# PJLab-ADG/neuralsim

Hardware: NVIDIA H100
Metric: Mrays/sec fwd+bwd (higher is better)
Workload: dtype f16

## Files before the change

neuralsim_b200/csrc/color_tc.cu:

```cuda
#include "fused_tc_common.cuh"
#include "sh_device.cuh"

namespace nsb {

struct ColorNetDev {
    DecoderDevTC dec;
    const __half *R1, *rb1, *R2, *rb2, *R3, *rb3;
    int rw, rin, n_appear;
    float fac[3];
};

constexpr int XW = 64;
constexpr int kTileBytes = kTile * XW * 2;
constexpr int kChunk = kTile * 16;

__host__ __device__ inline int ref_col(int k, int n_appear) {
    if (k < 32) return 22 + k;
    if (k < 35) return k - 32;
    if (k < 51) return 3 + (k - 35);
    if (k < 54) return 19 + (k - 51);
    if (k < 54 + n_appear) return k;
    return -1;
}


__device__ __forceinline__ void level_jacobian(const PLMeta &m, uint32_t p, const float (&xs)[3], const __half *__restrict__ grid,
                                               float (&J0)[3], float (&J1)[3]) {
    uint32_t cell[8];
    float w[8], fr[3], scale[3];
    level_cells3(m, p, xs, cell, w, fr, scale);
    const uint32_t *lp = level_cells_ptr(m, p, grid);
    float2 v[8];
#pragma unroll
    for (int c = 0; c < 8; ++c) {
        const uint32_t raw = ld_nc_u32(lp + cell[c]);
        v[c] = __half22float2(*reinterpret_cast<const __half2 *>(&raw));
    }
#pragma unroll
    for (int gd = 0; gd < 3; ++gd) {
        float a0 = 0.f, a1 = 0.f;
#pragma unroll
        for (int c = 0; c < 4; ++c) {
            float ww = scale[gd];
            int left = 0;
#pragma unroll
            for (int k = 0; k < 2; ++k) {
                const int d = k >= gd ? k + 1 : k;
                if (c & (1 << k)) { ww = __fmul_rn(ww, fr[d]); left += 1 << d; }
                else ww = __fmul_rn(ww, __fsub_rn(1.f, fr[d]));
            }
            const int right = left + (1 << gd);
            a0 = __fmaf_rn(ww, __fsub_rn(v[right].x, v[left].x), a0);
            a1 = __fmaf_rn(ww, __fsub_rn(v[right].y, v[left].y), a1);
        }
        J0[gd] = a0;
        J1[gd] = a1;
    }
}

__device__ __forceinline__ void unpack8(const uint4 &q, float (&v)[8]) {
    const __half2 *h = reinterpret_cast<const __half2 *>(&q);
#pragma unroll
    for (int i = 0; i < 4; ++i) { const float2 f = __half22float2(h[i]); v[2 * i] = f.x; v[2 * i + 1] = f.y; }
}

constexpr int kColorGatherU = 4;

constexpr int kColorBwdCtasPerSM = 2;

__global__ void __launch_bounds__(kTile)
k_color_fwd(const PLMeta m, const __half *__restrict__ grid, const ColorNetDev net, const PointSrc ps, const float *__restrict__ view_dirs,
            const float *__restrict__ h_appear, int64_t n, int max_level, float *__restrict__ sdf_out, float *__restrict__ nab_out,
            float *__restrict__ rgb_out, float *__restrict__ x_out, uint8_t *__restrict__ Zt, uint8_t *__restrict__ Xt,
            uint8_t *__restrict__ Y1t, uint8_t *__restrict__ Y2t, const OccCollect oc, const int64_t *__restrict__ n_dev) {
    n = eff_n(n, n_dev);
    extern __shared__ uint8_t dyn_smem[];
    uint8_t *tiles = reinterpret_cast<uint8_t *>((reinterpret_cast<uintptr_t>(dyn_smem) + 1023) & ~uintptr_t(1023));
    uint8_t *sX = tiles;
    uint8_t *sU = sX + kTileBytes;
    uint8_t *sW1 = sU + kTileBytes;
    uint8_t *sW1T = sW1 + HW * NF * 2;
    uint8_t *sR1 = sW1T + HW * NF * 2;
    uint8_t *sR2 = sR1 + XW * XW * 2;
    constexpr int kS = tc::acc_stride(64);
    float *acc = reinterpret_cast<float *>(sR2 + XW * XW * 2);
    __shared__ float sb1[HW], sW2[HW], srb1[XW], srb2[XW], sR3[3][XW];
    __shared__ float sb2, srb3[3];

    const int tid = threadIdx.x;
    stage_W1(net.dec, sW1, tid);
    stage_W1T(net.dec, sW1T, tid);
    for (int e = tid; e < XW * XW; e += kTile) {
        const int j = e % XW, k = e / XW;
        const int rc = ref_col(k, net.n_appear);
        const __half v1 = (j < net.rw && rc >= 0) ? net.R1[j * net.rin + rc] : __float2half_rn(0.f);
        const __half v2 = (j < net.rw && k < net.rw) ? net.R2[j * net.rw + k] : __float2half_rn(0.f);
        *reinterpret_cast<__half *>(sR1 + (k / 8) * (XW * 16) + j * 16 + (k % 8) * 2) = v1;
        *reinterpret_cast<__half *>(sR2 + (k / 8) * (XW * 16) + j * 16 + (k % 8) * 2) = v2;
    }
    stage_decoder_vectors(net.dec, sb1, sW2, &sb2, tid);
    if (tid < XW) {
        srb1[tid] = tid < net.rw ? __half2float(net.rb1[tid]) : 0.f;
        srb2[tid] = tid < net.rw ? __half2float(net.rb2[tid]) : 0.f;
#pragma unroll
        for (int k = 0; k < 3; ++k) sR3[k][tid] = tid < net.rw ? __half2float(net.R3[k * net.rw + tid]) : 0.f;
    }
    if (tid == 0) {
        for (int k = 0; k < 3; ++k) srb3[k] = __half2float(net.rb3[k]);
    }
    tc::fence_async_smem();
    __syncthreads();
    const uint32_t x_addr = tc::smem_u32(sX), u_addr = tc::smem_u32(sU), w1_addr = tc::smem_u32(sW1), w1t_addr = tc::smem_u32(sW1T);
    const uint32_t r1_addr = tc::smem_u32(sR1), r2_addr = tc::smem_u32(sR2);
    const SoftplusK spk(net.dec.beta);

    const int64_t n_tiles = (n + kTile - 1) / kTile;
    for (int64_t tile = blockIdx.x; tile < n_tiles; tile += gridDim.x) {
        const int64_t i = tile * kTile + tid;
        const bool valid = i < n;
        float xn[3], xs[3];
        int64_t ray;
        load_point(ps, ps.x == nullptr, i, valid, xn, xs, ray);
        gather_row_to_tile<kTile, kColorGatherU>(m, grid, xs, max_level, sX, tid);
        tc::fence_async_smem();
        __syncthreads();
        tc::mma_to_rows<64, 0, 0, NF / 16>(acc, kS, 0, tc::kmajor(x_addr, kTile), tc::kmajor(w1_addr, HW), false);
        __syncthreads();
        float out = 0.f;
        uint8_t *zt = Zt ? Zt + tile * kTileBytes : nullptr;
#pragma unroll 1
        for (int c = 0; c < HW / 8; ++c) {
            float z[8], uu[8];
            tc::acc_ld8(acc, kS, tid, c * 8, z);
#pragma unroll
            for (int j = 0; j < 8; ++j) {
                z[j] = r16(z[j] + sb1[c * 8 + j]);
                float a, s;
                softplus_as(z[j], spk, a, s);
                out = fmaf(r16(a), sW2[c * 8 + j], out);
                uu[j] = sW2[c * 8 + j] * s;
            }
            *reinterpret_cast<uint4 *>(sU + c * kChunk + tid * 16) = tc::pack8_f16(uu);
            if (zt) *reinterpret_cast<uint4 *>(zt + c * kChunk + tid * 16) = tc::pack8_f16(z);
        }
        const float sdf = r16(out + sb2);
        tc::fence_async_smem();
        __syncthreads();
        tc::mma_to_rows<32, 0, 0, HW / 16>(acc, kS, 0, tc::kmajor(u_addr, kTile), tc::kmajor(w1t_addr, NF), false);
        __syncthreads();
        float nacc[3] = {0.f, 0.f, 0.f};
#pragma unroll 1
        for (uint32_t g4 = 0; g4 < 4; ++g4) {
            float gg[8];
            tc::acc_ld8(acc, kS, tid, g4 * 8, gg);
#pragma unroll
            for (uint32_t q = 0; q < 4; ++q) {
                const uint32_t p = g4 * 4 + q;
                if ((int)m.level[p] <= max_level) {
                    float J0[3], J1[3];
                    level_jacobian(m, p, xs, grid, J0, J1);
                    const float g0 = r16(gg[2 * q]), g1 = r16(gg[2 * q + 1]);
#pragma unroll
                    for (int d = 0; d < 3; ++d) nacc[d] = __fmaf_rn(g0, J0[d], nacc[d]);
#pragma unroll
                    for (int d = 0; d < 3; ++d) nacc[d] = __fmaf_rn(g1, J1[d], nacc[d]);
                }
            }
        }
        float nab[3];
#pragma unroll
        for (int d = 0; d < 3; ++d) nab[d] = __fmul_rn(__fmul_rn(nacc[d], 0.5f), net.fac[d]);
        {
            float xr[32];
#pragma unroll
            for (int k = 0; k < 32; ++k) xr[k] = 0.f;
            xr[0] = xn[0]; xr[1] = xn[1]; xr[2] = xn[2];
            if (valid) {
                sh_basis(view_dirs[ray * 3], view_dirs[ray * 3 + 1], view_dirs[ray * 3 + 2], 4, xr + 3);
                if (h_appear) {
#pragma unroll
                    for (int k = 0; k < 8; ++k)
                        if (k < net.n_appear) xr[22 + k] = h_appear[ray * net.n_appear + k];
                }
            }
#pragma unroll
            for (int d = 0; d < 3; ++d) xr[19 + d] = fminf(fmaxf(nab[d], -1.f), 1.f);
            uint8_t *xt = Xt ? Xt + tile * kTileBytes : nullptr;
#pragma unroll
            for (int c = 0; c < 4; ++c) {
                float v8[8];
#pragma unroll
                for (int k = 0; k < 8; ++k) v8[k] = xr[c * 8 + k];
                const uint4 q = tc::pack8_f16(v8);
                *reinterpret_cast<uint4 *>(sX + (4 + c) * kChunk + tid * 16) = q;
                if (xt) {
                    *reinterpret_cast<uint4 *>(xt + (4 + c) * kChunk + tid * 16) = q;
                    *reinterpret_cast<uint4 *>(xt + c * kChunk + tid * 16) = *reinterpret_cast<const uint4 *>(sX + c * kChunk + tid * 16);
                }
            }
        }
        tc::fence_async_smem();
        __syncthreads();
        tc::mma_to_rows<64, 0, 0, XW / 16>(acc, kS, 0, tc::kmajor(x_addr, kTile), tc::kmajor(r1_addr, XW), false);
        __syncthreads();
        uint8_t *y1t = Y1t ? Y1t + tile * kTileBytes : nullptr;
#pragma unroll 1
        for (int c = 0; c < XW / 8; ++c) {
            float y[8];
            tc::acc_ld8(acc, kS, tid, c * 8, y);
#pragma unroll
            for (int j = 0; j < 8; ++j) y[j] = fmaxf(r16(y[j] + srb1[c * 8 + j]), 0.f);
            const uint4 q = tc::pack8_f16(y);
            *reinterpret_cast<uint4 *>(sU + c * kChunk + tid * 16) = q;
            if (y1t) *reinterpret_cast<uint4 *>(y1t + c * kChunk + tid * 16) = q;
        }
        tc::fence_async_smem();
        __syncthreads();
        tc::mma_to_rows<64, 0, 0, XW / 16>(acc, kS, 0, tc::kmajor(u_addr, kTile), tc::kmajor(r2_addr, XW), false);
        __syncthreads();
        float o3[3] = {0.f, 0.f, 0.f};
        uint8_t *y2t = Y2t ? Y2t + tile * kTileBytes : nullptr;
#pragma unroll 1
        for (int c = 0; c < XW / 8; ++c) {
            float y[8];
            tc::acc_ld8(acc, kS, tid, c * 8, y);
#pragma unroll
            for (int j = 0; j < 8; ++j) {
                y[j] = fmaxf(r16(y[j] + srb2[c * 8 + j]), 0.f);
#pragma unroll
                for (int k = 0; k < 3; ++k) o3[k] = fmaf(y[j], sR3[k][c * 8 + j], o3[k]);
            }
            if (y2t) *reinterpret_cast<uint4 *>(y2t + c * kChunk + tid * 16) = tc::pack8_f16(y);
        }
        if (valid) {
            sdf_out[i] = sdf;
            if (oc.pcl) occ_collect_point(oc, xs, sdf);
#pragma unroll
            for (int d = 0; d < 3; ++d) {
                nab_out[i * 3 + d] = nab[d];
                const float y3 = r16(o3[d] + srb3[d]);
                rgb_out[i * 3 + d] = r16(1.f / (1.f + expf(-y3)));
                if (x_out) x_out[i * 3 + d] = xn[d];
            }
        }
        __syncthreads();
    }
}

__global__ void __launch_bounds__(kTile, kColorBwdCtasPerSM)
k_color_rad_bwd(const ColorNetDev net, const uint8_t *__restrict__ Xt, const uint8_t *__restrict__ Y1t, const uint8_t *__restrict__ Y2t,
                const float *__restrict__ rgb, const float *__restrict__ g_rgb, int64_t n, float *__restrict__ dh_out,
                float *__restrict__ dR1, float *__restrict__ drb1, float *__restrict__ dR2, float *__restrict__ drb2,
                float *__restrict__ dR3, float *__restrict__ drb3, const int64_t *__restrict__ n_dev) {
    n = eff_n(n, n_dev);
    constexpr int NE = 80;
    extern __shared__ uint8_t dyn_smem[];
    uint8_t *tiles = reinterpret_cast<uint8_t *>((reinterpret_cast<uintptr_t>(dyn_smem) + 1023) & ~uintptr_t(1023));
    uint8_t *sT = tiles;
    uint8_t *sY1 = sT + 3 * kTileBytes;
    uint8_t *sXe = sY1 + kTile * NE * 2;
    uint8_t *sR2T = sXe + kTile * NE * 2;
    uint8_t *sR1h = sR2T + XW * XW * 2;
    __shared__ float sR3[3][XW];
    __shared__ float sdb3[3];
    __shared__ __align__(8) uint64_t mbar_ld;

    const int tid = threadIdx.x, lane = tid & 31;
    for (int e = tid; e < XW * XW; e += kTile) {
        const int i = e % XW, j = e / XW;
        const __half v = (j < net.rw && i < net.rw) ? net.R2[j * net.rw + i] : __float2half_rn(0.f);
        *reinterpret_cast<__half *>(sR2T + (j / 8) * (XW * 16) + i * 16 + (j % 8) * 2) = v;
    }
    for (int e = tid; e < NF * XW; e += kTile) {
        const int k = e % NF, j = e / NF;
        const __half v = j < net.rw ? net.R1[j * net.rin + 22 + k] : __float2half_rn(0.f);
        *reinterpret_cast<__half *>(sR1h + (j / 8) * (NF * 16) + k * 16 + (j % 8) * 2) = v;
    }
    if (tid < XW) {
#pragma unroll
        for (int k = 0; k < 3; ++k) sR3[k][tid] = tid < net.rw ? __half2float(net.R3[k * net.rw + tid]) : 0.f;
    }
    *reinterpret_cast<uint4 *>(sY1 + 8 * kChunk + tid * 16) = make_uint4(0x00003C00u, 0, 0, 0);
    *reinterpret_cast<uint4 *>(sY1 + 9 * kChunk + tid * 16) = make_uint4(0, 0, 0, 0);
    *reinterpret_cast<uint4 *>(sXe + 9 * kChunk + tid * 16) = make_uint4(0, 0, 0, 0);
    float xa[NE / 2], xb[NE / 2], x3[4];
#pragma unroll
    for (int k = 0; k < NE / 2; ++k) xa[k] = xb[k] = 0.f;
#pragma unroll
    for (int k = 0; k < 4; ++k) x3[k] = 0.f;
    if (tid == 0) {
        sdb3[0] = sdb3[1] = sdb3[2] = 0.f;
        tc::mbar_init(&mbar_ld, 1);
        tc::fence_mbar_init();
    }
    tc::fence_async_smem();
    __syncthreads();
    const uint32_t t_addr = tc::smem_u32(sT), y1_addr = tc::smem_u32(sY1), xe_addr = tc::smem_u32(sXe);
    const uint32_t r2t_addr = tc::smem_u32(sR2T), r1h_addr = tc::smem_u32(sR1h);
    uint32_t ld_phase = 0;
    bool first_tile = true;

    const int64_t n_tiles = (n + kTile - 1) / kTile;
    auto fetch = [&](int64_t tile) {
        tc::mbar_arrive_expect_tx(&mbar_ld, 3 * kTileBytes);
        tc::tma_load_bulk(sT + 2 * kTileBytes, Y2t + tile * kTileBytes, kTileBytes, &mbar_ld);
        tc::tma_load_bulk(sY1, Y1t + tile * kTileBytes, kTileBytes, &mbar_ld);
        tc::tma_load_bulk(sXe, Xt + tile * kTileBytes, kTileBytes, &mbar_ld);
    };
    if (tid == 0 && (int64_t)blockIdx.x < n_tiles) fetch(blockIdx.x);
    for (int64_t tile = blockIdx.x; tile < n_tiles; tile += gridDim.x) {
        const int64_t i = tile * kTile + tid;
        const bool valid = i < n;
        tc::mbar_wait(&mbar_ld, ld_phase);
        ld_phase ^= 1;
        float gy[3] = {0.f, 0.f, 0.f};
        if (valid && g_rgb) {
#pragma unroll
            for (int k = 0; k < 3; ++k) {
                const float y = rgb[i * 3 + k];
                gy[k] = r16(r16(g_rgb[i * 3 + k]) * ((1.f - y) * y));
            }
        }
        {
            float e8[8] = {1.f, gy[0], gy[1], gy[2], 0.f, 0.f, 0.f, 0.f};
            *reinterpret_cast<uint4 *>(sXe + 8 * kChunk + tid * 16) = tc::pack8_f16(e8);
        }
#pragma unroll
        for (int k = 0; k < 3; ++k) {
            const float sgy = warp_sum(gy[k]);
            if (lane == 0 && sgy != 0.f) atomicAdd(&sdb3[k], sgy);
        }
#pragma unroll 1
        for (int c = 0; c < 8; ++c) {
            float y2[8], d[8];
            unpack8(*reinterpret_cast<const uint4 *>(sT + 2 * kTileBytes + c * kChunk + tid * 16), y2);
#pragma unroll
            for (int j = 0; j < 8; ++j) {
                const float v = gy[0] * sR3[0][c * 8 + j] + gy[1] * sR3[1][c * 8 + j] + gy[2] * sR3[2][c * 8 + j];
                d[j] = y2[j] > 0.f ? v : 0.f;
            }
            *reinterpret_cast<uint4 *>(sT + c * kChunk + tid * 16) = tc::pack8_f16(d);
        }
        tc::fence_async_smem();
        __syncthreads();
        {
            float dy[2][XW / 2];
            tc::mma_m128<64, 0, 0, XW / 16>(dy, tc::kmajor(t_addr, kTile), tc::kmajor(r2t_addr, XW), false);
#pragma unroll
            for (int h = 0; h < 2; ++h)
#pragma unroll
                for (int c = 0; c < XW / 8; ++c)
#pragma unroll
                    for (int r = 0; r < 2; ++r) {
                        const uint32_t off = tc::pair_off<kTile>(h * 64 + tc::frag_row(r), tc::frag_col(c));
                        const float2 y1 = tc::ld_pair_f16(sY1, off);
                        tc::st_pair_f16(sT + kTileBytes, off, y1.x > 0.f ? dy[h][4 * c + 2 * r] : 0.f, y1.y > 0.f ? dy[h][4 * c + 2 * r + 1] : 0.f);
                    }
        }
        tc::fence_async_smem();
        __syncthreads();
        float dh[2][NF / 2];
        tc::mma_m128<32, 0, 0, XW / 16>(dh, tc::kmajor(t_addr + kTileBytes, kTile), tc::kmajor(r1h_addr, NF), false);
        tc::mma_m64<NE, 1, 1, kTile / 16>(xa, tc::mnmajor(t_addr, kTile), tc::mnmajor(y1_addr, kTile), true);
        tc::mma_m64<NE, 1, 1, kTile / 16>(xb, tc::mnmajor(t_addr + kTileBytes, kTile), tc::mnmajor(xe_addr, kTile), true);
        tc::mma_m64<8, 1, 1, kTile / 16>(x3, tc::mnmajor(t_addr + 2 * kTileBytes, kTile), tc::mnmajor(xe_addr + 8 * kChunk, kTile), true);
        first_tile = false;
        __syncthreads();
        if (tid == 0 && tile + gridDim.x < n_tiles) {
            tc::fence_async_smem();
            fetch(tile + gridDim.x);
        }
#pragma unroll
        for (int h = 0; h < 2; ++h)
#pragma unroll
            for (int r = 0; r < 2; ++r) {
                const int64_t row = tile * kTile + h * 64 + tc::frag_row(r);
                if (row < n) {
#pragma unroll
                    for (int c = 0; c < NF / 8; ++c)
                        *reinterpret_cast<float2 *>(dh_out + row * NF + tc::frag_col(c)) = make_float2(dh[h][4 * c + 2 * r], dh[h][4 * c + 2 * r + 1]);
                }
            }
    }
    if (!first_tile) {
#pragma unroll
        for (int r = 0; r < 2; ++r) {
            const int row = tc::frag_row(r);
            if (row >= net.rw) continue;
#pragma unroll
            for (int c = 0; c < NE / 8; ++c)
#pragma unroll
                for (int j = 0; j < 2; ++j) {
                    const int col = tc::frag_col(c) + j;
                    const float a = xa[4 * c + 2 * r + j], b = xb[4 * c + 2 * r + j];
                    if (col < XW) {
                        if (col < net.rw) atomicAdd(dR2 + row * net.rw + col, a);
                        const int rc = ref_col(col, net.n_appear);
                        if (rc >= 0) atomicAdd(dR1 + row * net.rin + rc, b);
                    } else if (col == XW) {
                        atomicAdd(drb2 + row, a);
                        atomicAdd(drb1 + row, b);
                    }
                }
#pragma unroll
            for (int j = 0; j < 2; ++j) {
                const int col = tc::frag_col(0) + j;
                if (col >= 1 && col <= 3) atomicAdd(dR3 + (col - 1) * net.rw + row, x3[2 * r + j]);
            }
        }
        if (tid < 3) atomicAdd(drb3 + tid, sdb3[tid]);
    }
}

__global__ void __launch_bounds__(kTile, kColorBwdCtasPerSM)
k_color_sdf_bwd(const PLMeta m, const __half *__restrict__ grid, const ColorNetDev net, const PointSrc ps, const uint8_t *__restrict__ Zt,
                const uint8_t *__restrict__ Xt, const float *__restrict__ g_nab, const float *__restrict__ g_sdf, const float *__restrict__ dh_r,
                int64_t n, int max_level, float *__restrict__ d_grid, float *__restrict__ d_W1, float *__restrict__ d_b1, float *__restrict__ d_W2,
                float *__restrict__ d_b2, const int64_t *__restrict__ n_dev) {
    n = eff_n(n, n_dev);
    constexpr int NX = 48;
    extern __shared__ uint8_t dyn_smem[];
    uint8_t *tiles = reinterpret_cast<uint8_t *>((reinterpret_cast<uintptr_t>(dyn_smem) + 1023) & ~uintptr_t(1023));
    uint8_t *sT = tiles;
    uint8_t *sHe = sT + 3 * kTileBytes;
    uint8_t *sGe = sHe + kTile * NX * 2;
    uint8_t *sW1 = sGe + kTile * NX * 2;
    uint8_t *sW1T = sW1 + HW * NF * 2;
    uint8_t *sZ = sW1T + NF * HW * 2;
    constexpr int kS = tc::acc_stride(2 * NF);
    float *stage = reinterpret_cast<float *>(sT);
    static_assert(kTile * kS * 4 <= 3 * kTileBytes, "the staged rows must fit in T");
    __shared__ float sW2[HW], sdsdf[kTile];
    __shared__ float sdb2;
    __shared__ __align__(8) uint64_t mbar_ld;

    const int tid = threadIdx.x, lane = tid & 31;
    stage_W1(net.dec, sW1, tid);
    stage_W1T(net.dec, sW1T, tid);
    stage_decoder_vectors(net.dec, nullptr, sW2, nullptr, tid);
    *reinterpret_cast<uint4 *>(sHe + 4 * kChunk + tid * 16) = make_uint4(0x00003C00u, 0, 0, 0);
    *reinterpret_cast<uint4 *>(sGe + 4 * kChunk + tid * 16) = make_uint4(0x00003C00u, 0, 0, 0);
    *reinterpret_cast<uint4 *>(sHe + 5 * kChunk + tid * 16) = make_uint4(0, 0, 0, 0);
    *reinterpret_cast<uint4 *>(sGe + 5 * kChunk + tid * 16) = make_uint4(0, 0, 0, 0);
    float wacc[NX / 2], vacc[4];
#pragma unroll
    for (int k = 0; k < NX / 2; ++k) wacc[k] = 0.f;
#pragma unroll
    for (int k = 0; k < 4; ++k) vacc[k] = 0.f;
    if (tid == 0) {
        sdb2 = 0.f;
        tc::mbar_init(&mbar_ld, 1);
        tc::fence_mbar_init();
    }
    tc::fence_async_smem();
    __syncthreads();
    const uint32_t t_addr = tc::smem_u32(sT), he_addr = tc::smem_u32(sHe), ge_addr = tc::smem_u32(sGe), w1_addr = tc::smem_u32(sW1),
                   w1t_addr = tc::smem_u32(sW1T);
    const SoftplusK spk(net.dec.beta);
    uint32_t ld_phase = 0;
    bool first_tile = true;

    const int64_t n_tiles = (n + kTile - 1) / kTile;
    auto fetch = [&](int64_t tile) {
        tc::mbar_arrive_expect_tx(&mbar_ld, kTileBytes + 4 * kChunk);
        tc::tma_load_bulk(sZ, Zt + tile * kTileBytes, kTileBytes, &mbar_ld);
        tc::tma_load_bulk(sHe, Xt + tile * kTileBytes, 4 * kChunk, &mbar_ld);
    };
    if (tid == 0 && (int64_t)blockIdx.x < n_tiles) fetch(blockIdx.x);
    for (int64_t tile = blockIdx.x; tile < n_tiles; tile += gridDim.x) {
        const int64_t i = tile * kTile + tid;
        const bool valid = i < n;
        float xn[3], xs[3];
        int64_t ray;
        load_point(ps, ps.x == nullptr, i, valid, xn, xs, ray);
        float gin[3] = {0.f, 0.f, 0.f};
        if (valid && g_nab) {
#pragma unroll
            for (int d = 0; d < 3; ++d) gin[d] = g_nab[i * 3 + d] * net.fac[d] * 0.5f;
        }
        const float dsdf = (valid && g_sdf) ? g_sdf[i] : 0.f;
        sdsdf[tid] = dsdf;
        tc::mbar_wait(&mbar_ld, ld_phase);
        ld_phase ^= 1;
#pragma unroll 1
        for (int c = 0; c < 8; ++c) {
            float z[8], uu[8];
            unpack8(*reinterpret_cast<const uint4 *>(sZ + c * kChunk + tid * 16), z);
#pragma unroll
            for (int j = 0; j < 8; ++j) {
                float a, s;
                softplus_as(z[j], spk, a, s);
                uu[j] = sW2[c * 8 + j] * s;
            }
            *reinterpret_cast<uint4 *>(sT + kTileBytes + c * kChunk + tid * 16) = tc::pack8_f16(uu);
        }
#pragma unroll 4
        for (uint32_t p = 0; p < 16; ++p) {
            uint32_t packed = 0;
            if ((int)m.level[p] <= max_level) {
                float J0[3], J1[3];
                level_jacobian(m, p, xs, grid, J0, J1);
                float a0 = 0.f, a1 = 0.f;
#pragma unroll
                for (int d = 0; d < 3; ++d) { a0 = __fmaf_rn(gin[d], J0[d], a0); a1 = __fmaf_rn(gin[d], J1[d], a1); }
                const __half2 h = __floats2half2_rn(a0, a1);
                packed = *reinterpret_cast<const uint32_t *>(&h);
            }
            *reinterpret_cast<uint32_t *>(sGe + (p >> 2) * kChunk + tid * 16 + (p & 3) * 4) = packed;
        }
        tc::fence_async_smem();
        __syncthreads();
        float gfr[2][NF / 2];
        {
            float du[2][HW / 2];
            tc::mma_m128<64, 0, 0, NF / 16>(du, tc::kmajor(ge_addr, kTile), tc::kmajor(w1_addr, HW), false);
            tc::mma_m128<32, 0, 0, HW / 16>(gfr, tc::kmajor(t_addr + kTileBytes, kTile), tc::kmajor(w1t_addr, NF), false);
#pragma unroll
            for (int h = 0; h < 2; ++h)
#pragma unroll
                for (int r = 0; r < 2; ++r) {
                    const int row = h * 64 + tc::frag_row(r);
                    const float ds = sdsdf[row];
#pragma unroll
                    for (int c = 0; c < HW / 8; ++c) {
                        const int col = tc::frag_col(c);
                        const uint32_t off = tc::pair_off<kTile>(row, col);
                        const float2 z2 = tc::ld_pair_f16(sZ, off);
                        float dz[2], vv[2];
#pragma unroll
                        for (int j = 0; j < 2; ++j) {
                            const float z = j ? z2.y : z2.x;
                            float a, s;
                            softplus_as(z, spk, a, s);
                            const float w2 = sW2[col + j], d = r16(du[h][4 * c + 2 * r + j]);
                            const float curv = (z * spk.k > spk.thr) ? 0.f : spk.beta * s * (1.f - s);
                            dz[j] = d * w2 * curv + ds * w2 * s;
                            vv[j] = d * s + ds * r16(a);
                        }
                        tc::st_pair_f16(sT, off, dz[0], dz[1]);
                        tc::st_pair_f16(sT + 2 * kTileBytes, off, vv[0], vv[1]);
                    }
                }
        }
        tc::fence_async_smem();
        __syncthreads();
        float dhz[2][NF / 2];
        tc::mma_m128<32, 0, 0, HW / 16>(dhz, tc::kmajor(t_addr, kTile), tc::kmajor(w1t_addr, NF), false);
        tc::mma_m64<NX, 1, 1, kTile / 16>(wacc, tc::mnmajor(t_addr, kTile), tc::mnmajor(he_addr, kTile), true);
        tc::mma_m64<NF, 1, 1, kTile / 16>(*reinterpret_cast<float(*)[NF / 2]>(wacc), tc::mnmajor(t_addr + kTileBytes, kTile), tc::mnmajor(ge_addr, kTile), true);
        tc::mma_m64<8, 1, 1, kTile / 16>(vacc, tc::mnmajor(t_addr + 2 * kTileBytes, kTile), tc::mnmajor(ge_addr + 4 * kChunk, kTile), true);
        first_tile = false;
        const float dsum = warp_sum(dsdf);
        if (lane == 0 && dsum != 0.f) atomicAdd(&sdb2, dsum);
        __syncthreads();
        if (tid == 0 && tile + gridDim.x < n_tiles) {
            tc::fence_async_smem();
            fetch(tile + gridDim.x);
        }
        tc::frag_store<NF>(gfr, stage, kS, 0);
        tc::frag_store<NF>(dhz, stage, kS, NF);
        __syncthreads();
#pragma unroll 1
        for (uint32_t g4 = 0; g4 < 4; ++g4) {
            float gg[8], hz[8];
            tc::acc_ld8(stage, kS, tid, g4 * 8, gg);
            tc::acc_ld8(stage, kS, tid, NF + g4 * 8, hz);
            if (valid && dh_r) {
                const float4 r0 = *reinterpret_cast<const float4 *>(dh_r + i * NF + g4 * 8), r1 = *reinterpret_cast<const float4 *>(dh_r + i * NF + g4 * 8 + 4);
                hz[0] += r0.x; hz[1] += r0.y; hz[2] += r0.z; hz[3] += r0.w; hz[4] += r1.x; hz[5] += r1.y; hz[6] += r1.z; hz[7] += r1.w;
            }
#pragma unroll
            for (uint32_t q = 0; q < 4; ++q) {
                const uint32_t p = g4 * 4 + q;
                if ((int)m.level[p] > max_level) continue;
                uint32_t cell[8];
                float w[8], fr[3], sc[3], ua[8], ub[8];
                level_cells3(m, p, xs, cell, w, fr, sc);
                const float g0 = valid ? r16(gg[2 * q]) : 0.f, g1 = valid ? r16(gg[2 * q + 1]) : 0.f;
                const float h0 = valid ? hz[2 * q] : 0.f, h1 = valid ? hz[2 * q + 1] : 0.f;
#pragma unroll
                for (int c = 0; c < 8; ++c) {
                    float wsum = 0.f;
#pragma unroll
                    for (int gd = 0; gd < 3; ++gd) {
                        float ww = __fmul_rn(sc[gd], gin[gd]);
#pragma unroll
                        for (int d = 0; d < 3; ++d) {
                            if (d == gd) continue;
                            ww = __fmul_rn(ww, (c & (1 << d)) ? fr[d] : __fsub_rn(1.f, fr[d]));
                        }
                        wsum += (c & (1 << gd)) ? ww : -ww;
                    }
                    ua[c] = g0 * wsum + h0 * w[c];
                    ub[c] = g1 * wsum + h1 * w[c];
                }
                bool issue = valid;
                if (level_mergeable(m, p)) issue = warp_merge_updates(cell_key3(m, p, xs), valid, ua, ub, lane);
                if (issue) {
                    float2 *gp = level_grad_ptr(m, p, d_grid);
#pragma unroll
                    for (int c = 0; c < 8; ++c) red_add2(gp + cell[c], ua[c], ub[c]);
                }
            }
        }
        __syncthreads();
    }
    if (!first_tile) {
#pragma unroll
        for (int r = 0; r < 2; ++r) {
            const int row = tc::frag_row(r);
            if (row >= net.dec.width) continue;
#pragma unroll
            for (int c = 0; c <= NF / 8; ++c)
#pragma unroll
                for (int j = 0; j < 2; ++j) {
                    const int col = tc::frag_col(c) + j;
                    if (col < NF) atomicAdd(d_W1 + row * NF + col, wacc[4 * c + 2 * r + j]);
                    else if (col == NF) atomicAdd(d_b1 + row, wacc[4 * c + 2 * r + j]);
                }
            if (tc::frag_col(0) == 0) atomicAdd(d_W2 + row, vacc[2 * r]);
        }
        if (tid == 0) atomicAdd(d_b2, sdb2);
    }
}

}

using namespace nsb;

namespace {
int make_net(const nsb_color_net *c, const nsb_lotd_meta *meta, PLMeta *m, ColorNetDev *d, const char *who) {
    const nsb_sdf_decoder dec{c->W1, c->b1, c->W2, c->b2, c->width, c->beta};
    if (int rc = make_decoder(meta, &dec, m, &d->dec, who)) return rc;
    NSB_REQUIRE(c->rad_width >= 1 && c->rad_width <= 64, "%s: radiance width must be <= 64", who);
    NSB_REQUIRE(c->n_appear >= 0 && c->n_appear <= 8 && c->rad_in == 54 + c->n_appear,
                "%s: radiance input must be [x(3), SH deg 4 (16), n(3), h(32), h_appear(<=8)]", who);
    d->R1 = (const __half *)c->R1; d->rb1 = (const __half *)c->rb1; d->R2 = (const __half *)c->R2; d->rb2 = (const __half *)c->rb2;
    d->R3 = (const __half *)c->R3; d->rb3 = (const __half *)c->rb3;
    d->rw = c->rad_width; d->rin = c->rad_in; d->n_appear = c->n_appear;
    for (int k = 0; k < 3; ++k) d->fac[k] = c->nablas_scale[k];
    return 0;
}
}

static int64_t n_tiles(int64_t n) { return (n + kTile - 1) / kTile; }

extern "C" int64_t nsb_color_tile_bytes(int64_t n) { return n_tiles(n) * (int64_t)kTileBytes; }

extern "C" int nsb_fused_color_fwd(const nsb_lotd_meta *meta, const void *params_half, const nsb_color_net *net, const float *x, const float *rays_o,
                                   const float *rays_d, const int64_t *ridx, const float *t, const float *view_dirs, const float *h_appear,
                                   int64_t n, int32_t max_level, float *sdf, float *nablas, float *rgb, float *x_out, void *act_z, void *act_x,
                                   void *act_y1, void *act_y2, const nsb_occ_collect *collect, void *stream) {
    const DevCounts dn = take_counts();
    if (n == 0) return 0;
    NSB_REQUIRE(meta && params_half && net && sdf && nablas && rgb && view_dirs, "nsb_fused_color_fwd: NULL argument");
    NSB_REQUIRE(x || (rays_o && rays_d && t), "nsb_fused_color_fwd: need x or (rays_o, rays_d, t)");
    NSB_REQUIRE((act_z && act_x && act_y1 && act_y2) || (!act_z && !act_x && !act_y1 && !act_y2), "nsb_fused_color_fwd: pass all four activation buffers or none");
    PLMeta m;
    ColorNetDev d;
    if (int rc = make_net(net, meta, &m, &d, "nsb_fused_color_fwd")) return rc;
    NSB_REQUIRE(d.n_appear == 0 || h_appear, "nsb_fused_color_fwd: h_appear is NULL but the net has %d appearance channels", d.n_appear);
    constexpr int kSmem = 2 * kTileBytes + 2 * HW * NF * 2 + 2 * XW * XW * 2 + kTile * tc::acc_stride(64) * 4 + 1024;
    opt_in_smem(k_color_fwd, kSmem);
    const PointSrc ps{x, rays_o, rays_d, t, ridx};
    k_color_fwd<<<persistent_grid(n_tiles(n), 2), kTile, kSmem, (cudaStream_t)stream>>>(m, (const __half *)params_half, d, ps, view_dirs, h_appear, n,
                                                                                        max_level < 0 ? -1 : max_level, sdf, nablas, rgb, x_out, (uint8_t *)act_z,
                                                                                        (uint8_t *)act_x, (uint8_t *)act_y1, (uint8_t *)act_y2,
                                                                                        occ_collect_of(collect), dn.a);
    return check_launch("nsb_fused_color_fwd");
}

extern "C" int nsb_fused_color_bwd(const nsb_lotd_meta *meta, const void *params_half, const nsb_color_net *net, const float *x, const float *rays_o,
                                   const float *rays_d, const int64_t *ridx, const float *t, int64_t n, int32_t max_level, const void *act_z,
                                   const void *act_x, const void *act_y1, const void *act_y2, const float *rgb, const float *g_sdf,
                                   const float *g_nablas, const float *g_rgb, float *dh_scratch, float *d_grid, float *d_W1, float *d_b1,
                                   float *d_W2, float *d_b2, float *d_R1, float *d_rb1, float *d_R2, float *d_rb2, float *d_R3, float *d_rb3,
                                   void *stream) {
    const DevCounts dn = take_counts();
    if (n == 0) return 0;
    NSB_REQUIRE(meta && params_half && net && act_z && act_x && act_y1 && act_y2 && rgb && dh_scratch, "nsb_fused_color_bwd: NULL argument");
    NSB_REQUIRE(d_grid && d_W1 && d_b1 && d_W2 && d_b2 && d_R1 && d_rb1 && d_R2 && d_rb2 && d_R3 && d_rb3, "nsb_fused_color_bwd: NULL gradient buffer");
    NSB_REQUIRE(x || (rays_o && rays_d && t), "nsb_fused_color_bwd: need x or (rays_o, rays_d, t)");
    PLMeta m;
    ColorNetDev d;
    if (int rc = make_net(net, meta, &m, &d, "nsb_fused_color_bwd")) return rc;
    cudaStream_t s = (cudaStream_t)stream;
    const float *dh = nullptr;
    if (g_rgb) {
        constexpr int kSmemR = 3 * kTileBytes + 2 * kTile * 80 * 2 + XW * XW * 2 + NF * XW * 2 + 1024;
        opt_in_smem(k_color_rad_bwd, kSmemR);
        if (int rc = require_ctas_per_sm(k_color_rad_bwd, kTile, kSmemR, kColorBwdCtasPerSM, "nsb_fused_color_bwd(radiance)")) return rc;
        k_color_rad_bwd<<<persistent_grid(n_tiles(n), kColorBwdCtasPerSM), kTile, kSmemR, s>>>(d, (const uint8_t *)act_x, (const uint8_t *)act_y1,
                                                                                               (const uint8_t *)act_y2, rgb, g_rgb, n, dh_scratch, d_R1,
                                                                                               d_rb1, d_R2, d_rb2, d_R3, d_rb3, dn.a);
        if (int rc = check_launch("nsb_fused_color_bwd(radiance)")) return rc;
        dh = dh_scratch;
    }
    constexpr int kSmemS = 3 * kTileBytes + 2 * kTile * 48 * 2 + 2 * HW * NF * 2 + kTileBytes + 1024;
    opt_in_smem(k_color_sdf_bwd, kSmemS);
    if (int rc = require_ctas_per_sm(k_color_sdf_bwd, kTile, kSmemS, kColorBwdCtasPerSM, "nsb_fused_color_bwd(sdf)")) return rc;
    const PointSrc ps{x, rays_o, rays_d, t, ridx};
    k_color_sdf_bwd<<<persistent_grid(n_tiles(n), kColorBwdCtasPerSM), kTile, kSmemS, s>>>(m, (const __half *)params_half, d, ps, (const uint8_t *)act_z, (const uint8_t *)act_x,
                                                                          g_nablas, g_sdf, dh, n, max_level < 0 ? -1 : max_level, d_grid, d_W1, d_b1, d_W2, d_b2, dn.a);
    return check_launch("nsb_fused_color_bwd(sdf)");
}
```

neuralsim_b200/csrc/fused_tc_common.cuh:

```cuda
#pragma once
#include "lotd_device.cuh"
#include "tc_util.cuh"

namespace nsb {

struct DecoderDevTC {
    const __half *W1, *b1, *W2, *b2;
    int width;
    float beta;
};

struct OccCollect {
    float *pcl;
    int rx, ry, rz;
    float inv_s;
};
inline OccCollect occ_collect_of(const nsb_occ_collect *c) {
    if (c && c->grid_pcl) return OccCollect{c->grid_pcl, c->res[0], c->res[1], c->res[2], c->inv_s};
    return OccCollect{nullptr, 1, 1, 1, 0.f};
}
__device__ __forceinline__ float r16(float v) { return __half2float(__float2half_rn(v)); }
__device__ __forceinline__ void occ_collect_point(const OccCollect &oc, const float (&xs)[3], float sdf) {
    const int ix = min(max((int)__fmul_rn(xs[0], (float)oc.rx), 0), oc.rx - 1);
    const int iy = min(max((int)__fmul_rn(xs[1], (float)oc.ry), 0), oc.ry - 1);
    const int iz = min(max((int)__fmul_rn(xs[2], (float)oc.rz), 0), oc.rz - 1);
    const float a = fminf(fmaxf(r16(r16(__fmul_rn(sdf, oc.inv_s)) * 0.5f), -20.f), 20.f);
    const float r = r16(__fdiv_rn(1.f, r16(coshf(a))));
    const float v = r16(__fmul_rn(r, r));
    if (v > 0.f) atomicMax(reinterpret_cast<int *>(oc.pcl) + ((ix * oc.ry + iy) * oc.rz + iz), __float_as_int(v));
}

constexpr int kTile = 128;
constexpr int NF = 32, HW = 64;

template <int R, int U = 2>
__device__ __forceinline__ void gather_row_to_tile(const PLMeta &m, const __half *__restrict__ grid, const float (&xs)[3],
                                                   int max_level, uint8_t *tile, int r) {
#pragma unroll 1
    for (uint32_t p0 = 0; p0 < 16; p0 += U) {
        uint32_t cell[U][8];
        float w[U][8];
        uint32_t packed[U];
#pragma unroll
        for (int u = 0; u < U; ++u) level_cells3(m, p0 + u, xs, cell[u], w[u]);
#pragma unroll
        for (int u = 0; u < U; ++u) packed[u] = level_feat2_cells(level_cells_ptr(m, p0 + u, grid), cell[u], w[u]);
#pragma unroll
        for (int u = 0; u < U; ++u) {
            const uint32_t p = p0 + u;
            *reinterpret_cast<uint32_t *>(tile + (p >> 2) * (R * 16) + r * 16 + (p & 3) * 4) = ((int)m.level[p] <= max_level) ? packed[u] : 0u;
        }
    }
}

struct PointSrc {
    const float *x, *rays_o, *rays_d, *t;
    const int64_t *ridx;
};

__device__ __forceinline__ void load_point(const PointSrc &ps, bool from_rays, int64_t i, bool valid, float (&xn)[3], float (&xs)[3],
                                           int64_t &ray) {
    xn[0] = xn[1] = xn[2] = 0.f;
    ray = 0;
    if (valid) {
        if (from_rays) {
            ray = ps.ridx ? ps.ridx[i] : i;
            const float tt = ps.t[i];
#pragma unroll
            for (int d = 0; d < 3; ++d) xn[d] = __fmaf_rn(ps.rays_d[ray * 3 + d], tt, ps.rays_o[ray * 3 + d]);
        } else {
#pragma unroll
            for (int d = 0; d < 3; ++d) xn[d] = ps.x[i * 3 + d];
            ray = ps.ridx ? ps.ridx[i] : i;
        }
    }
#pragma unroll
    for (int d = 0; d < 3; ++d) xs[d] = to_table_space(xn[d]);
}
__device__ __forceinline__ void load_point(const PointSrc &ps, bool from_rays, int64_t i, bool valid, float (&xs)[3]) {
    float xn[3];
    int64_t ray;
    load_point(ps, from_rays, i, valid, xn, xs, ray);
}

struct SoftplusK {
    float k, thr, out;
    float beta;
    __device__ __forceinline__ explicit SoftplusK(float b) : k(b * 1.4426950408889634f), thr(20.f * 1.4426950408889634f), out(0.6931471805599453f / b), beta(b) {}
};
__device__ __forceinline__ float ex2_approx(float x) { float r; asm("ex2.approx.ftz.f32 %0, %1;" : "=f"(r) : "f"(x)); return r; }
__device__ __forceinline__ float lg2_approx(float x) { float r; asm("lg2.approx.ftz.f32 %0, %1;" : "=f"(r) : "f"(x)); return r; }
__device__ __forceinline__ float rcp_approx(float x) { float r; asm("rcp.approx.ftz.f32 %0, %1;" : "=f"(r) : "f"(x)); return r; }

__device__ __forceinline__ float softplus_a(float zz, const SoftplusK &K) {
    const float t = zz * K.k;
    const float e = ex2_approx(t);
    const float a = lg2_approx(1.f + e) * K.out;
    return t > K.thr ? zz : a;
}
__device__ __forceinline__ void softplus_as(float zz, const SoftplusK &K, float &a, float &s) {
    const float t = zz * K.k;
    const float e = ex2_approx(t);
    const float d = 1.f + e;
    const bool lin = t > K.thr;
    a = lin ? zz : lg2_approx(d) * K.out;
    s = lin ? 1.f : e * rcp_approx(d);
}

__device__ __forceinline__ void stage_W1(const DecoderDevTC &dec, uint8_t *sB, int tid) {
    for (int e = tid; e < HW * (NF / 8); e += kTile) {
        const int j = e % HW, c = e / HW;
        uint4 q = make_uint4(0, 0, 0, 0);
        if (j < dec.width) q = *reinterpret_cast<const uint4 *>(dec.W1 + j * NF + c * 8);
        *reinterpret_cast<uint4 *>(sB + c * (HW * 16) + j * 16) = q;
    }
}

__device__ __forceinline__ void stage_W1T(const DecoderDevTC &dec, uint8_t *sBT, int tid) {
    for (int e = tid; e < NF * HW; e += kTile) {
        const int k = e % NF, j = e / NF;
        const __half v = j < dec.width ? dec.W1[j * NF + k] : __float2half_rn(0.f);
        *reinterpret_cast<__half *>(sBT + (j / 8) * (NF * 16) + k * 16 + (j % 8) * 2) = v;
    }
}

template <typename B1, typename B2>
__device__ __forceinline__ void stage_decoder_vectors(const DecoderDevTC &dec, B1 sb1, float *sW2, B2 sb2, int tid) {
    constexpr bool kB1 = !std::is_same<B1, std::nullptr_t>::value, kB2 = !std::is_same<B2, std::nullptr_t>::value;
    if (tid < HW) {
        if constexpr (kB1) sb1[tid] = tid < dec.width ? __half2float(dec.b1[tid]) : 0.f;
        sW2[tid] = tid < dec.width ? __half2float(dec.W2[tid]) : 0.f;
    }
    if constexpr (kB2) {
        if (tid == 0) *sb2 = __half2float(dec.b2[0]);
    }
}

inline int make_decoder(const nsb_lotd_meta *meta, const nsb_sdf_decoder *dec, PLMeta *m, DecoderDevTC *d, const char *who) {
    if (make_plmeta(meta, m)) return 2;
    NSB_REQUIRE(m->n_pseudo == 16 && m->F == 2 && m->D == 3 && plmeta_two_feature_cells(*m), "%s: built for 16 x 2 LoTD features in 3-D", who);
    NSB_REQUIRE(dec->width >= 1 && dec->width <= 64, "%s: decoder width must be <= 64", who);
    *d = DecoderDevTC{(const __half *)dec->W1, (const __half *)dec->b1, (const __half *)dec->W2, (const __half *)dec->b2, dec->width, dec->beta};
    return 0;
}

struct SdfTile {
    const PLMeta &m;
    const __half *grid;
    int max_level;
    uint8_t *sA;
    uint32_t a_addr, b_addr;
    float *srow;
    const float *sb1, *sW2;
    float sb2;
    SoftplusK spk;
};

__device__ __forceinline__ float sdf_of_tile(const SdfTile &c, const float (&xs)[3], int tid) {
    gather_row_to_tile<kTile>(c.m, c.grid, xs, c.max_level, c.sA, tid);
    tc::fence_async_smem();
    __syncthreads();
    float z[2][HW / 2];
    tc::mma_m128<HW, 0, 0, NF / 16>(z, tc::kmajor(c.a_addr, kTile), tc::kmajor(c.b_addr, HW), false);
    const int lane = tid & 31, q = lane & 3;
#pragma unroll
    for (int h = 0; h < 2; ++h)
#pragma unroll
        for (int i = 0; i < 2; ++i) {
            float out = 0.f;
#pragma unroll
            for (int ch = 0; ch < HW / 8; ++ch)
#pragma unroll
                for (int j = 0; j < 2; ++j) {
                    const int col = ch * 8 + 2 * q + j;
                    const float zz = r16(z[h][4 * ch + 2 * i + j] + c.sb1[col]);
                    out = fmaf(r16(softplus_a(zz, c.spk)), c.sW2[col], out);
                }
            out += __shfl_xor_sync(0xffffffffu, out, 1);
            out += __shfl_xor_sync(0xffffffffu, out, 2);
            if (q == 0) c.srow[h * 64 + (tid >> 5) * 16 + (lane >> 2) + 8 * i] = out;
        }
    __syncthreads();
    return r16(c.srow[tid] + c.sb2);
}

}
```

neuralsim_b200/csrc/lotd_device.cuh:

```cuda
#pragma once
#include <type_traits>

#include "nsb_common.cuh"

namespace nsb {

constexpr int kMaxPseudo = 32;

struct PLMeta {
    uint32_t n_pseudo, n_out, D, F;
    uint32_t level[kMaxPseudo];
    uint32_t res[kMaxPseudo][NSB_MAX_DIMS];
    uint32_t base[kMaxPseudo];
    uint32_t nfeat[kMaxPseudo];
    uint32_t size[kMaxPseudo];
    uint32_t mask[kMaxPseudo];
    uint32_t is_hash;
};

inline int make_plmeta(const nsb_lotd_meta *m, PLMeta *o) {
    if (m->n_pseudo_levels > (uint32_t)kMaxPseudo) {
        set_error("LoTD: %u pseudo levels exceed the built maximum %d", m->n_pseudo_levels, kMaxPseudo);
        return 2;
    }
    memset(o, 0, sizeof(*o));
    o->n_pseudo = m->n_pseudo_levels;
    o->n_out = m->n_encoded_dims;
    o->D = m->n_dims_to_encode;
    o->F = m->n_feat_per_pseudo_lvl;
    for (uint32_t p = 0; p < m->n_pseudo_levels; ++p) {
        const uint32_t l = m->map_levels[p];
        o->level[p] = l;
        for (int d = 0; d < NSB_MAX_DIMS; ++d) o->res[p][d] = m->level_res[l][d];
        o->base[p] = m->level_offsets[l] + m->map_cnt[p] * m->n_feat_per_pseudo_lvl;
        o->nfeat[p] = m->level_n_feats[l];
        o->size[p] = m->level_sizes[l];
        o->mask[p] = (o->size[p] & (o->size[p] - 1)) == 0 ? o->size[p] - 1 : 0;
        if (m->level_types[l] == NSB_LOD_HASH) {
            if (p >= 32) { set_error("LoTD: hashed pseudo level index >= 32 unsupported"); return 2; }
            o->is_hash |= (1u << p);
        }
    }
    return 0;
}

template <bool HALF> struct ValT { using type = float; };
template <> struct ValT<true> { using type = __half; };

__device__ __forceinline__ float to_float(float v) { return v; }
__device__ __forceinline__ float to_float(__half v) { return __half2float(v); }
template <typename T> __device__ __forceinline__ T from_float(float v);
template <> __device__ __forceinline__ float from_float<float>(float v) { return v; }
template <> __device__ __forceinline__ __half from_float<__half>(float v) { return __float2half_rn(v); }
template <typename T> __device__ __forceinline__ T add_st(T a, T b);
template <> __device__ __forceinline__ float add_st<float>(float a, float b) { return __fadd_rn(a, b); }
template <> __device__ __forceinline__ __half add_st<__half>(__half a, __half b) { return __hadd(a, b); }

__device__ __forceinline__ float to_table_space(float x) { return fminf(fmaxf(__fmaf_rn(x, 0.5f, 0.5f), 1.0e-6f), 1.f - 1.0e-6f); }

template <int D>
__device__ __forceinline__ void level_pos(const PLMeta &m, uint32_t p, const float (&xs)[D], uint32_t (&cell)[D],
                                          float (&fr)[D], float (&scale)[D]) {
#pragma unroll
    for (int d = 0; d < D; ++d) {
        scale[d] = (float)(m.res[p][d] - 2u);
        const float v = __fmaf_rn(xs[d], scale[d], 0.5f);
        const float fl = floorf(v);
        cell[d] = (uint32_t)fl;
        fr[d] = v - fl;
    }
}

template <int D>
__device__ __forceinline__ float corner_weight(const float (&fr)[D], int c) {
    float w = (c & 1) ? fr[0] : __fsub_rn(1.f, fr[0]);
#pragma unroll
    for (int d = 1; d < D; ++d) w = __fmul_rn(w, (c & (1 << d)) ? fr[d] : __fsub_rn(1.f, fr[d]));
    return w;
}

template <int D>
__device__ __forceinline__ uint32_t corner_index(const PLMeta &m, uint32_t p, const uint32_t (&cell)[D], int c) {
    uint32_t idx;
    if (m.is_hash & (1u << p)) {
        constexpr uint32_t primes[4] = {1u, 2654435761u, 805459861u, 3674653429u};
        idx = 0;
#pragma unroll
        for (int d = 0; d < D; ++d) idx ^= (cell[d] + ((c >> d) & 1)) * primes[d];
        idx %= m.size[p];
    } else {
        idx = 0;
        uint32_t stride = 1;
#pragma unroll
        for (int d = D - 1; d >= 0; --d) {
            idx += (cell[d] + ((c >> d) & 1)) * stride;
            stride *= m.res[p][d];
        }
    }
    return idx * m.nfeat[p] + m.base[p];
}

template <int D, int F, typename VT>
__device__ __forceinline__ void load_corner(const PLMeta &m, uint32_t p, const VT *__restrict__ grid,
                                            const uint32_t (&cell)[D], int c, VT (&out)[F]) {
    const uint32_t e = corner_index<D>(m, p, cell, c);
    if constexpr (std::is_same<VT, __half>::value) {
#pragma unroll
        for (int f = 0; f < F; f += 2) {
            const uint32_t raw = ld_nc_u32(grid + e + f);
            out[f] = __ushort_as_half((unsigned short)(raw & 0xffffu));
            out[f + 1] = __ushort_as_half((unsigned short)(raw >> 16));
        }
    } else {
#pragma unroll
        for (int f = 0; f < F; ++f) out[f] = __ldg(grid + e + f);
    }
}

__device__ __forceinline__ void level_corners3(const PLMeta &m, uint32_t p, const float (&xs)[3], uint32_t (&idx)[8], float (&w)[8]) {
    const uint32_t rx = m.res[p][0], ry = m.res[p][1], rz = m.res[p][2];
    uint32_t cell[3];
    float fr[3];
    {
        const float sx = (float)(rx - 2u), sy = (float)(ry - 2u), sz = (float)(rz - 2u);
        const float vx = __fmaf_rn(xs[0], sx, 0.5f), vy = __fmaf_rn(xs[1], sy, 0.5f), vz = __fmaf_rn(xs[2], sz, 0.5f);
        const float fx = floorf(vx), fy = floorf(vy), fz = floorf(vz);
        cell[0] = (uint32_t)fx; cell[1] = (uint32_t)fy; cell[2] = (uint32_t)fz;
        fr[0] = vx - fx; fr[1] = vy - fy; fr[2] = vz - fz;
    }
    const float wx0 = __fsub_rn(1.f, fr[0]), wy0 = __fsub_rn(1.f, fr[1]), wz0 = __fsub_rn(1.f, fr[2]);
    const float w00 = __fmul_rn(wx0, wy0), w10 = __fmul_rn(fr[0], wy0), w01 = __fmul_rn(wx0, fr[1]), w11 = __fmul_rn(fr[0], fr[1]);
    w[0] = __fmul_rn(w00, wz0); w[1] = __fmul_rn(w10, wz0); w[2] = __fmul_rn(w01, wz0); w[3] = __fmul_rn(w11, wz0);
    w[4] = __fmul_rn(w00, fr[2]); w[5] = __fmul_rn(w10, fr[2]); w[6] = __fmul_rn(w01, fr[2]); w[7] = __fmul_rn(w11, fr[2]);
    const uint32_t nf = m.nfeat[p], base = m.base[p];
    if (m.is_hash & (1u << p)) {
        const uint32_t hx0 = cell[0], hx1 = cell[0] + 1u;
        const uint32_t hy0 = cell[1] * 2654435761u, hy1 = hy0 + 2654435761u;
        const uint32_t hz0 = cell[2] * 805459861u, hz1 = hz0 + 805459861u;
        const uint32_t a00 = hy0 ^ hz0, a10 = hy1 ^ hz0, a01 = hy0 ^ hz1, a11 = hy1 ^ hz1;
        uint32_t h[8] = {hx0 ^ a00, hx1 ^ a00, hx0 ^ a10, hx1 ^ a10, hx0 ^ a01, hx1 ^ a01, hx0 ^ a11, hx1 ^ a11};
        const uint32_t mask = m.mask[p], size = m.size[p];
#pragma unroll
        for (int c = 0; c < 8; ++c) idx[c] = (mask ? (h[c] & mask) : (h[c] % size)) * nf + base;
    } else {
        const uint32_t sy_ = rz, sx_ = ry * rz;
        const uint32_t b0 = (cell[0] * ry + cell[1]) * rz + cell[2];
#pragma unroll
        for (int c = 0; c < 8; ++c) idx[c] = (b0 + ((c & 1) ? sx_ : 0u) + ((c & 2) ? sy_ : 0u) + ((c & 4) ? 1u : 0u)) * nf + base;
    }
}

__device__ __forceinline__ void level_cells3(const PLMeta &m, uint32_t p, const float (&xs)[3], uint32_t (&cell)[8], float (&w)[8],
                                             float (&fr)[3], float (&sc)[3]) {
    const uint32_t rx = m.res[p][0], ry = m.res[p][1], rz = m.res[p][2];
    sc[0] = (float)(rx - 2u); sc[1] = (float)(ry - 2u); sc[2] = (float)(rz - 2u);
    const float vx = __fmaf_rn(xs[0], sc[0], 0.5f), vy = __fmaf_rn(xs[1], sc[1], 0.5f), vz = __fmaf_rn(xs[2], sc[2], 0.5f);
    const float tx = __fadd_rd(vx, 8388608.f), ty = __fadd_rd(vy, 8388608.f), tz = __fadd_rd(vz, 8388608.f);
    const uint32_t cx = __float_as_uint(tx) - 0x4B000000u, cy = __float_as_uint(ty) - 0x4B000000u, cz = __float_as_uint(tz) - 0x4B000000u;
    fr[0] = vx - (tx - 8388608.f); fr[1] = vy - (ty - 8388608.f); fr[2] = vz - (tz - 8388608.f);
    const float wx0 = __fsub_rn(1.f, fr[0]), wy0 = __fsub_rn(1.f, fr[1]), wz0 = __fsub_rn(1.f, fr[2]);
    const float w00 = __fmul_rn(wx0, wy0), w10 = __fmul_rn(fr[0], wy0), w01 = __fmul_rn(wx0, fr[1]), w11 = __fmul_rn(fr[0], fr[1]);
    w[0] = __fmul_rn(w00, wz0); w[1] = __fmul_rn(w10, wz0); w[2] = __fmul_rn(w01, wz0); w[3] = __fmul_rn(w11, wz0);
    w[4] = __fmul_rn(w00, fr[2]); w[5] = __fmul_rn(w10, fr[2]); w[6] = __fmul_rn(w01, fr[2]); w[7] = __fmul_rn(w11, fr[2]);
    if (m.is_hash & (1u << p)) {
        const uint32_t hx0 = cx, hx1 = cx + 1u;
        const uint32_t hy0 = cy * 2654435761u, hy1 = hy0 + 2654435761u;
        const uint32_t hz0 = cz * 805459861u, hz1 = hz0 + 805459861u;
        const uint32_t a00 = hy0 ^ hz0, a10 = hy1 ^ hz0, a01 = hy0 ^ hz1, a11 = hy1 ^ hz1;
        const uint32_t h[8] = {hx0 ^ a00, hx1 ^ a00, hx0 ^ a10, hx1 ^ a10, hx0 ^ a01, hx1 ^ a01, hx0 ^ a11, hx1 ^ a11};
        const uint32_t mask = m.mask[p];
        if (mask) {
#pragma unroll
            for (int c = 0; c < 8; ++c) cell[c] = h[c] & mask;
        } else {
            const uint32_t size = m.size[p];
#pragma unroll
            for (int c = 0; c < 8; ++c) cell[c] = h[c] % size;
        }
    } else {
        const uint32_t sy_ = rz, sx_ = ry * rz;
        const uint32_t b0 = (cx * ry + cy) * rz + cz;
        cell[0] = b0; cell[1] = b0 + sx_; cell[2] = b0 + sy_; cell[3] = cell[1] + sy_;
        cell[4] = b0 + 1u; cell[5] = cell[1] + 1u; cell[6] = cell[2] + 1u; cell[7] = cell[3] + 1u;
    }
}

__device__ __forceinline__ void level_cells3(const PLMeta &m, uint32_t p, const float (&xs)[3], uint32_t (&cell)[8], float (&w)[8]) {
    float fr[3], sc[3];
    level_cells3(m, p, xs, cell, w, fr, sc);
}

__device__ __forceinline__ const uint32_t *level_cells_ptr(const PLMeta &m, uint32_t p, const __half *grid) {
    const uint32_t *q = reinterpret_cast<const uint32_t *>(grid + m.base[p]);
    asm volatile("" : "+l"(q));
    return q;
}
__device__ __forceinline__ float2 *level_grad_ptr(const PLMeta &m, uint32_t p, float *d_grid) {
    float2 *q = reinterpret_cast<float2 *>(d_grid + m.base[p]);
    asm volatile("" : "+l"(q));
    return q;
}

__device__ __forceinline__ uint32_t level_feat2_cells(const uint32_t *__restrict__ lp, const uint32_t (&cell)[8], const float (&w)[8]) {
    uint32_t raw[8];
#pragma unroll
    for (int c = 0; c < 8; ++c) raw[c] = ld_nc_u32(lp + cell[c]);
    __half2 acc = __floats2half2_rn(0.f, 0.f);
#pragma unroll
    for (int c = 0; c < 8; ++c) {
        const float2 v = __half22float2(*reinterpret_cast<const __half2 *>(&raw[c]));
        acc = __hadd2(acc, __floats2half2_rn(__fmul_rn(w[c], v.x), __fmul_rn(w[c], v.y)));
    }
    return *reinterpret_cast<uint32_t *>(&acc);
}

__device__ __forceinline__ void red_add2(float2 *dst, float a, float b) {
    asm volatile("red.global.add.v2.f32 [%0], {%1, %2};" ::"l"(dst), "f"(a), "f"(b) : "memory");
}

__device__ __forceinline__ uint32_t cell_key3(const PLMeta &m, uint32_t p, const float (&xs)[3]) {
    uint32_t k = 0;
#pragma unroll
    for (int d = 0; d < 3; ++d) {
        const float v = __fmaf_rn(xs[d], (float)(m.res[p][d] - 2u), 0.5f);
        k |= (__float_as_uint(__fadd_rd(v, 8388608.f)) - 0x4B000000u) << (10 * d);
    }
    return k;
}
__device__ __forceinline__ bool level_mergeable(const PLMeta &m, uint32_t p) {
    return m.res[p][0] <= 1024u && m.res[p][1] <= 1024u && m.res[p][2] <= 1024u;
}

__device__ __forceinline__ bool warp_merge_updates(uint32_t key, bool active, float (&a)[8], float (&b)[8], int lane) {
    const uint32_t prev = __shfl_up_sync(0xffffffffu, key, 1);
    const uint32_t act = __ballot_sync(0xffffffffu, active);
    const bool prev_act = lane > 0 && ((act >> (lane - 1)) & 1u);
    const bool head = !active || !prev_act || key != prev;
    const uint32_t heads = __ballot_sync(0xffffffffu, head);
    if (__popc(heads) > 24) return active;
    const uint32_t after = lane == 31 ? 0xffffffffu : (heads >> (lane + 1));
#pragma unroll
    for (int o = 1; o < 32; o <<= 1) {
        const bool take = (lane + o < 32) && ((after & ((1u << o) - 1u)) == 0u);
#pragma unroll
        for (int c = 0; c < 8; ++c) {
            const float av = __shfl_down_sync(0xffffffffu, a[c], o), bv = __shfl_down_sync(0xffffffffu, b[c], o);
            if (take) { a[c] += av; b[c] += bv; }
        }
    }
    return active && head;
}

inline bool plmeta_two_feature_cells(const PLMeta &m) {
    for (uint32_t p = 0; p < m.n_pseudo; ++p)
        if (m.nfeat[p] != 2u || (m.base[p] & 1u)) return false;
    return m.F == 2u;
}

template <int F>
__device__ __forceinline__ void red_add(float *dst, const float (&g)[F], float w) {
#pragma unroll
    for (int f = 0; f < F; f += 2) {
        const float a = g[f] * w, b = g[f + 1] * w;
        asm volatile("red.global.add.v2.f32 [%0], {%1, %2};" ::"l"(dst + f), "f"(a), "f"(b) : "memory");
    }
}

}
```

neuralsim_b200/fields/fused_color.py:

```python
from __future__ import annotations

import ctypes

import torch
from torch import autograd

from .. import _lib as L


class _FusedColor(autograd.Function):
    @staticmethod
    def forward(ctx, model, pts, view_dirs, h_appear, max_level, keep, collect, *params):
        grid16, net, _held = model._fused_color_state()
        ridx, t, rays_o, rays_d = pts
        n, dev = t.numel(), t.device
        meta = model.implicit_surface.encoding.meta
        sdf = torch.empty(n, dtype=torch.float32, device=dev)
        nab = torch.empty(n, 3, dtype=torch.float32, device=dev)
        rgb = torch.empty(n, 3, dtype=torch.float32, device=dev)
        x = torch.empty(n, 3, dtype=torch.float32, device=dev)
        acts = None
        if keep:
            acts = torch.empty(4, int(L.lib().nsb_color_tile_bytes(L.c_i64(n))), dtype=torch.uint8, device=dev)
        ap = [L.ptr(acts[k]) if keep else None for k in range(4)]
        with L.KERNEL_TIMER.time("fused_color_fwd", n):
            L.check(L.lib().nsb_fused_color_fwd(meta.c_ref, L.ptr(grid16, "f16"), ctypes.byref(net), None, L.ptr(rays_o, "f32"), L.ptr(rays_d, "f32"),
                                                L.ptr(ridx, "i64"), L.ptr(t, "f32"), L.ptr(view_dirs, "f32"), L.ptr(h_appear, "f32", allow_none=True),
                                                L.c_i64(n), L.c_i32(max_level), L.ptr(sdf), L.ptr(nab), L.ptr(rgb), L.ptr(x), *ap,
                                                ctypes.byref(collect) if collect is not None else None, L.stream_ptr()),
                    "fused_color_fwd")
        ctx.model, ctx.pts, ctx.max_level, ctx.n = model, pts, max_level, n
        ctx.held = (grid16, net, _held, acts, rgb)
        ctx.shapes = [p.shape for p in params]
        ctx.set_materialize_grads(False)
        ctx.mark_non_differentiable(x)
        return sdf, nab, rgb, x

    @staticmethod
    @autograd.function.once_differentiable
    def backward(ctx, g_sdf, g_nab, g_rgb, _gx):
        grid16, net, _held, acts, rgb = ctx.held
        if acts is None:
            raise RuntimeError("fused_color: backward through a forward that ran without grad")
        dev, n = rgb.device, ctx.n
        meta = ctx.model.implicit_surface.encoding.meta
        sizes = [int(torch.Size(s).numel()) for s in ctx.shapes[1:]]
        small = torch.zeros(sum(sizes), dtype=torch.float32, device=dev)
        grads, o = [torch.zeros(ctx.shapes[0], dtype=torch.float32, device=dev)], 0
        for sh, k in zip(ctx.shapes[1:], sizes):
            grads.append(small[o:o + k].view(sh))
            o += k
        if g_sdf is None and g_nab is None and g_rgb is None:
            return (None,) * 7 + tuple(grads)
        ridx, t, rays_o, rays_d = ctx.pts
        c = lambda g: None if g is None else g.contiguous().float()
        g_sdf, g_nab, g_rgb = c(g_sdf), c(g_nab), c(g_rgb)
        dh = torch.empty(n, 32, dtype=torch.float32, device=dev)
        with L.KERNEL_TIMER.time("fused_color_bwd", n):
            L.check(L.lib().nsb_fused_color_bwd(meta.c_ref, L.ptr(grid16, "f16"), ctypes.byref(net), None, L.ptr(rays_o, "f32"), L.ptr(rays_d, "f32"),
                                                L.ptr(ridx, "i64"), L.ptr(t, "f32"), L.c_i64(n), L.c_i32(ctx.max_level), L.ptr(acts[0]), L.ptr(acts[1]),
                                                L.ptr(acts[2]), L.ptr(acts[3]), L.ptr(rgb), L.ptr(g_sdf, allow_none=True), L.ptr(g_nab, allow_none=True),
                                                L.ptr(g_rgb, allow_none=True), L.ptr(dh), *[L.ptr(g) for g in grads], L.stream_ptr()),
                    "fused_color_bwd")
        return (None,) * 7 + tuple(grads)


def fused_color(model, ridx, t, rays_o, rays_d, view_dirs, h_appear=None, *, nablas_has_grad=True, collect=None):
    s, r = model.implicit_surface, model.radiance_net.blocks.layers
    d = s.decoder.layers
    params = (s.encoding.flattened_params, d[0].weight, d[0].bias, d[1].weight, d[1].bias, r[0].weight, r[0].bias, r[1].weight, r[1].bias,
              r[2].weight, r[2].bias)
    pts = (ridx.reshape(-1).contiguous().long(), t.detach().reshape(-1).contiguous().float(), rays_o.detach().contiguous().float(),
           rays_d.detach().contiguous().float())
    keep = torch.is_grad_enabled() and any(p.requires_grad for p in params)
    ha = None if h_appear is None else h_appear.detach().contiguous().float()
    sdf, nab, rgb, x = _FusedColor.apply(model, pts, view_dirs.detach().contiguous().float(), ha, s._ml(model.max_level), keep, collect, *params)
    if not nablas_has_grad:
        nab = nab.detach()
    return dict(sdf=sdf, nablas=nab, rgb=rgb, x=x)
```

neuralsim_b200/graphics/neus_static.py:

```python
from __future__ import annotations

import ctypes

import torch
import torch.nn.functional as F

from .. import _lib as L
from .raysample import batch_sample_step_linear
from .pack_ops import get_pack_infos_from_batch
from . import neus_fused as NF

__all__ = ["render_static", "StaticFrame", "CNT_SLOTS"]

CNT_SLOTS = dict(n_rays=0, pairs=2, marched_raw=3, hit_raw=4, kept_raw=6, kept_rays_raw=7, nonzero=9, marched=12, hit=13, fine0=14,
                 boundary=18, kept=19, overflow=20, kept_rays=21, merged0=22, rays_if_kept_fits=26, row_len=27)
_NULL = ctypes.c_void_p(0)
MARCH_ONEPASS = "auto"
MARCH_ONEPASS_MAX_BYTES = 64 << 20


def march_onepass(n_rays, max_steps):
    if MARCH_ONEPASS == "0":
        return False
    return MARCH_ONEPASS == "1" or 4 * int(n_rays) * int(max_steps) <= MARCH_ONEPASS_MAX_BYTES


def _slot(cnt, k):
    return ctypes.c_void_p(cnt.data_ptr() + 8 * k)


def _call(fn, what, cnt, k0, k1, *args):
    lib = L.lib()
    lib.nsb_bind_device_counts(_slot(cnt, k0), _slot(cnt, k1) if k1 is not None else _NULL)
    try:
        rc = fn(*args)
    finally:
        lib.nsb_bind_device_counts(_NULL, _NULL)
    L.check(rc, what)


def _scan(counts, cnt, slot, *, first=None, info2=None, index=None, pack=None, src=None, nz_src=None, ws=None):
    if ws is None:
        ws = torch.zeros(NF._scan_ws_bytes(), dtype=torch.uint8, device=counts.device)
    P = L.ptr
    L.check(L.lib().nsb_scan_counts(P(counts, "i32"), L.c_i64(counts.shape[0]), P(first, allow_none=True), P(info2, allow_none=True),
                                    P(index, allow_none=True), P(pack, allow_none=True), P(src, "i64", allow_none=True), P(nz_src, allow_none=True),
                                    _slot(cnt, slot), None, L.c_i64(0), P(ws), L.stream_ptr()), "scan_counts")


def _query_counts(cnt, phase, n_coarse1, num_fine, march_cap, kept_cap):
    nf = (ctypes.c_int32 * max(len(num_fine), 1))(*[int(n) for n in num_fine])
    L.check(L.lib().nsb_query_counts(ctypes.c_void_p(cnt.data_ptr()), L.c_i32(phase), L.c_i32(n_coarse1), nf, L.c_i32(len(num_fine)),
                                     L.c_i64(march_cap), L.c_i64(kept_cap), L.stream_ptr()), "query_counts")


def _sdf_launch(meta, grid16, dec, rays_o, rays_d, t, sdf, *, ridx=None, packs=None, ml, collect, cnt, slot, timer="lotd_gather"):
    P = L.ptr
    mode = 2 if packs is not None else 1
    with L.KERNEL_TIMER.time(timer, t.numel()):
        _call(L.lib().nsb_fused_sdf_collect, "fused_sdf", cnt, slot, None,
              meta.c_ref, P(grid16, "f16"), ctypes.byref(dec), None, P(rays_o, "f32"), P(rays_d, "f32"),
              P(ridx, "i64") if mode == 1 else None, P(t, "f32"), L.c_i64(t.numel()),
              P(packs[0], "i64") if mode == 2 else None, P(packs[1], "i64", allow_none=True) if mode == 2 else None,
              P(packs[2], "i64", allow_none=True) if mode == 2 and len(packs) > 2 else None,
              L.c_i64(packs[0].shape[0] if mode == 2 else 0), L.c_i32(mode), L.c_i32(ml), P(sdf),
              ctypes.byref(collect) if collect is not None else None, L.stream_ptr())
    return sdf


def _block_order(rays_inds, via, n_rays, cnt, slot):
    n = rays_inds.shape[0] if via is None else via.shape[0]
    order = torch.empty(n, dtype=torch.int64, device=rays_inds.device)
    _call(L.lib().nsb_ray_block_order, "ray_block_order", cnt, slot, None, L.ptr(rays_inds, "i64"), L.ptr(via, "i64", allow_none=True), L.c_i64(n),
          L.c_i64(n_rays), _slot(cnt, CNT_SLOTS["pairs"]), _slot(cnt, CNT_SLOTS["row_len"]), L.ptr(order), L.stream_ptr())
    return order


class _StaticSDF(torch.autograd.Function):

    @staticmethod
    def forward(ctx, st, ridx, t, packs, count_slot, grid, W1, b1, W2, b2):
        sdf = torch.empty(t.numel(), dtype=torch.float32, device=t.device)
        _sdf_launch(st.meta, st.grid16, st.dec, st.rays_o, st.rays_d, t, sdf, ridx=ridx if packs is None else None, packs=packs, ml=st.ml,
                    collect=st.collect, cnt=st.cnt, slot=count_slot, timer="fused_sdf_fwd")
        ctx.st, ctx.ridx, ctx.t = st, ridx, t
        ctx.shapes = (grid.shape, W1.shape, b1.shape, W2.shape, b2.shape)
        return sdf

    @staticmethod
    @torch.autograd.function.once_differentiable
    def backward(ctx, d_sdf):
        st, dev = ctx.st, d_sdf.device
        gs, w1s, b1s, w2s, b2s = ctx.shapes
        d_grid = torch.zeros(gs, dtype=torch.float32, device=dev)
        ks = [int(torch.Size(x).numel()) for x in (w1s, b1s, w2s, b2s)]
        small = torch.zeros(sum(ks), dtype=torch.float32, device=dev)
        d_W1, d_b1 = small[:ks[0]].view(w1s), small[ks[0]:ks[0] + ks[1]].view(b1s)
        d_W2, d_b2 = small[ks[0] + ks[1]:ks[0] + ks[1] + ks[2]].view(w2s), small[ks[0] + ks[1] + ks[2]:].view(b2s)
        d_sdf = d_sdf.contiguous().float()
        n = d_sdf.numel()
        P, cnt = L.ptr, st.cnt
        flag = torch.empty(n, dtype=torch.int32, device=dev)
        _call(L.lib().nsb_flag_nonzero, "flag_nonzero", cnt, CNT_SLOTS["boundary"], None, P(d_sdf, "f32"), L.c_i64(n), P(flag), L.stream_ptr())
        keep = torch.empty(n, dtype=torch.int64, device=dev)
        _scan(flag, cnt, CNT_SLOTS["nonzero"], index=keep, ws=st.ws[3])
        with L.KERNEL_TIMER.time("fused_sdf_bwd", n):
            _call(L.lib().nsb_fused_sdf_bwd_indexed, "fused_sdf_bwd", cnt, CNT_SLOTS["nonzero"], None,
                  st.meta.c_ref, P(st.grid16, "f16"), ctypes.byref(st.dec), None, P(st.rays_o, "f32"), P(st.rays_d, "f32"), P(ctx.ridx, "i64"),
                  P(ctx.t, "f32"), P(d_sdf, "f32"), P(keep, "i64"), L.c_i64(n), L.c_i32(st.ml), P(d_grid), P(d_W1), P(d_b1), P(d_W2), P(d_b2),
                  L.stream_ptr())
        return None, None, None, None, None, d_grid, d_W1, d_b1, d_W2, d_b2


class _StaticAlpha(torch.autograd.Function):

    @staticmethod
    def forward(ctx, sdf, inv_s, pack_infos, cnt, early_stop_eps, alpha_thre):
        sdf_c, inv_c = sdf.detach().contiguous().float(), inv_s.detach().contiguous().float().reshape(1)
        Pn, dev = pack_infos.shape[0], sdf_c.device
        alpha = torch.empty_like(sdf_c)
        sel = torch.empty(sdf_c.shape[0], dtype=torch.bool, device=dev)
        steps = torch.empty(Pn, dtype=torch.int32, device=dev)
        P = L.ptr
        _call(L.lib().nsb_neus_alpha_forward, "neus_alpha_forward", cnt, CNT_SLOTS["n_rays"], None, P(sdf_c, "f32"), P(pack_infos, "i64"), L.c_i64(Pn),
              P(inv_c, "f32"), L.c_f32(early_stop_eps), L.c_f32(alpha_thre), P(alpha), P(sel), P(steps), L.stream_ptr())
        ctx.save_for_backward(sdf_c, inv_c, pack_infos)
        ctx.cnt, ctx.inv_shape = cnt, inv_s.shape
        ctx.mark_non_differentiable(sel, steps)
        return alpha, sel, steps

    @staticmethod
    def backward(ctx, g_alpha, _gs, _gn):
        sdf_c, inv_c, pack_infos = ctx.saved_tensors
        g = g_alpha.contiguous().float()
        d_sdf = torch.empty_like(sdf_c)
        d_inv = torch.zeros(1, device=sdf_c.device, dtype=torch.float32)
        P = L.ptr
        _call(L.lib().nsb_neus_alpha_backward, "neus_alpha_backward", ctx.cnt, CNT_SLOTS["n_rays"], None, P(sdf_c, "f32"), P(pack_infos, "i64"),
              L.c_i64(pack_infos.shape[0]), P(inv_c, "f32"), P(g, "f32"), P(d_sdf), P(d_inv), L.stream_ptr())
        return (d_sdf if ctx.needs_input_grad[0] else None, d_inv.reshape(ctx.inv_shape) if ctx.needs_input_grad[1] else None, None, None, None, None)


class _StaticGather(torch.autograd.Function):

    @staticmethod
    def forward(ctx, src, pidx, gathered, cnt):
        ctx.save_for_backward(pidx)
        ctx.n, ctx.cnt = src.shape[0], cnt
        return gathered

    @staticmethod
    def backward(ctx, g):
        pidx, = ctx.saved_tensors
        g = g.contiguous().float()
        d = torch.zeros(ctx.n, dtype=torch.float32, device=g.device)
        P = L.ptr
        _call(L.lib().nsb_scatter_f32, "scatter_f32", ctx.cnt, CNT_SLOTS["kept"], None, P(g, "f32"), P(pidx, "i64"), L.c_i64(pidx.shape[0]), P(d), L.stream_ptr())
        return d, None, None, None


class _StaticColor(torch.autograd.Function):

    @staticmethod
    def forward(ctx, st, ridx, t, view_dirs, h_appear, keep_acts, *params):
        n, dev = t.numel(), t.device
        sdf = torch.empty(n, dtype=torch.float32, device=dev)
        nab = torch.empty(n, 3, dtype=torch.float32, device=dev)
        rgb = torch.empty(n, 3, dtype=torch.float32, device=dev)
        x = torch.empty(n, 3, dtype=torch.float32, device=dev)
        acts = torch.empty(4, int(L.lib().nsb_color_tile_bytes(L.c_i64(n))), dtype=torch.uint8, device=dev) if keep_acts else None
        ap = [L.ptr(acts[k]) if keep_acts else None for k in range(4)]
        P = L.ptr
        with L.KERNEL_TIMER.time("fused_color_fwd", n):
            _call(L.lib().nsb_fused_color_fwd, "fused_color_fwd", st.cnt, CNT_SLOTS["kept"], None,
                  st.meta.c_ref, P(st.grid16, "f16"), ctypes.byref(st.net), None, P(st.rays_o, "f32"), P(st.rays_d, "f32"), P(ridx, "i64"), P(t, "f32"),
                  P(view_dirs, "f32"), P(h_appear, "f32", allow_none=True), L.c_i64(n), L.c_i32(st.ml), P(sdf), P(nab), P(rgb), P(x), *ap,
                  ctypes.byref(st.collect) if st.collect is not None else None, L.stream_ptr())
        ctx.st, ctx.ridx, ctx.t, ctx.n = st, ridx, t, n
        ctx.held = (acts, rgb)
        ctx.shapes = [p.shape for p in params]
        ctx.set_materialize_grads(False)
        ctx.mark_non_differentiable(x)
        return sdf, nab, rgb, x

    @staticmethod
    @torch.autograd.function.once_differentiable
    def backward(ctx, g_sdf, g_nab, g_rgb, _gx):
        acts, rgb = ctx.held
        if acts is None:
            raise RuntimeError("static colour query: backward through a forward that ran without grad")
        st, dev, n = ctx.st, rgb.device, ctx.n
        sizes = [int(torch.Size(s).numel()) for s in ctx.shapes[1:]]
        small = torch.zeros(sum(sizes), dtype=torch.float32, device=dev)
        grads, o = [torch.zeros(ctx.shapes[0], dtype=torch.float32, device=dev)], 0
        for sh, k in zip(ctx.shapes[1:], sizes):
            grads.append(small[o:o + k].view(sh))
            o += k
        if g_sdf is None and g_nab is None and g_rgb is None:
            return (None,) * 6 + tuple(grads)
        c = lambda g: None if g is None else g.contiguous().float()
        g_sdf, g_nab, g_rgb = c(g_sdf), c(g_nab), c(g_rgb)
        dh = torch.empty(n, 32, dtype=torch.float32, device=dev)
        P = L.ptr
        with L.KERNEL_TIMER.time("fused_color_bwd", n):
            _call(L.lib().nsb_fused_color_bwd, "fused_color_bwd", st.cnt, CNT_SLOTS["kept"], None,
                  st.meta.c_ref, P(st.grid16, "f16"), ctypes.byref(st.net), None, P(st.rays_o, "f32"), P(st.rays_d, "f32"), P(ctx.ridx, "i64"),
                  P(ctx.t, "f32"), L.c_i64(n), L.c_i32(st.ml), P(acts[0]), P(acts[1]), P(acts[2]), P(acts[3]), P(rgb), P(g_sdf, allow_none=True),
                  P(g_nab, allow_none=True), P(g_rgb, allow_none=True), P(dh), *[P(g) for g in grads], L.stream_ptr())
        return (None,) * 6 + tuple(grads)


class _StaticComposite(torch.autograd.Function):

    @staticmethod
    def forward(ctx, alpha, t, rgb, nablas, pack_infos, ray_index, n_rays, cnt, normalize_depth, early_stop_eps, alpha_thre):
        a, tt = alpha.detach().contiguous().float(), t.detach().contiguous().float()
        r = None if rgb is None else rgb.detach().contiguous().float()
        nb = None if nablas is None else nablas.detach().contiguous().float()
        Pn, dev = pack_infos.shape[0], a.device
        vw = torch.empty_like(a)
        cols = 2 + (3 if r is not None else 0) + (3 if nb is not None else 0)
        buf = torch.zeros(cols * n_rays, device=dev)
        mask, depth = buf[:n_rays], buf[n_rays:2 * n_rays]
        rgb_o = buf[2 * n_rays:5 * n_rays].view(n_rays, 3) if r is not None else None
        o3 = 5 * n_rays if r is not None else 2 * n_rays
        nab_o = buf[o3:o3 + 3 * n_rays].view(n_rays, 3) if nb is not None else None
        P = L.ptr
        _call(L.lib().nsb_composite_forward, "composite_forward", cnt, CNT_SLOTS["kept_rays"], None, P(a, "f32"), P(tt, "f32"), P(r, "f32", allow_none=True),
              P(nb, "f32", allow_none=True), P(pack_infos, "i64"), L.c_i64(Pn), L.c_f32(early_stop_eps), L.c_f32(alpha_thre),
              ctypes.c_int(1 if normalize_depth else 0), P(ray_index, "i64"), P(vw), P(mask), P(depth), P(rgb_o, allow_none=True),
              P(nab_o, allow_none=True), L.stream_ptr())
        ctx.save_for_backward(a, tt, r, nb, vw, pack_infos, mask, depth, ray_index)
        ctx.cfg = (normalize_depth, early_stop_eps, alpha_thre, cnt)
        ctx.set_materialize_grads(False)
        empty = a.new_empty(0)
        return vw, mask, depth, (rgb_o if rgb_o is not None else empty), (nab_o if nab_o is not None else empty)

    @staticmethod
    def backward(ctx, g_vw, g_mask, g_depth, g_rgb, g_nab):
        a, tt, r, nb, vw, pack_infos, mask, depth, ray_index = ctx.saved_tensors
        normalize_depth, eps, thre, cnt = ctx.cfg

        def opt(g, present=True):
            return None if (g is None or not present) else g.contiguous().float()
        g_vw, g_mask, g_depth = opt(g_vw), opt(g_mask), opt(g_depth)
        g_rgb, g_nab = opt(g_rgb, r is not None), opt(g_nab, nb is not None)
        d_alpha = torch.empty_like(a)
        d_rgb = torch.empty_like(r) if r is not None else None
        d_nab = torch.empty_like(nb) if nb is not None else None
        P = L.ptr
        _call(L.lib().nsb_composite_backward, "composite_backward", cnt, CNT_SLOTS["kept_rays"], None,
              P(a, "f32"), P(tt, "f32"), P(r, allow_none=True), P(nb, allow_none=True), P(vw, "f32"), P(pack_infos, "i64"), L.c_i64(pack_infos.shape[0]),
              L.c_f32(eps), L.c_f32(thre), ctypes.c_int(1 if normalize_depth else 0), P(mask), P(depth), P(g_mask, allow_none=True),
              P(g_depth, allow_none=True), P(g_rgb, allow_none=True), P(g_nab, allow_none=True), P(g_vw, allow_none=True), P(ray_index, "i64"),
              P(d_alpha), P(d_rgb, allow_none=True), P(d_nab, allow_none=True), L.stream_ptr())
        return (d_alpha, None, d_rgb, d_nab) + (None,) * 7


class _State:
    __slots__ = ("meta", "grid16", "dec", "net", "held", "rays_o", "rays_d", "ml", "collect", "cnt", "ws")


def _fp16_images(model):
    s, b = model.implicit_surface, model.radiance_net.blocks.layers
    d = s.decoder.layers
    ps = [s.encoding.flattened_params, d[0].weight, d[0].bias, d[1].weight, d[1].bias, b[0].weight, b[0].bias, b[1].weight, b[1].bias, b[2].weight, b[2].bias]
    t = [torch.empty(p.shape, dtype=torch.half, device=p.device) for p in ps]
    with torch.no_grad():
        t[0].copy_(ps[0].detach())
        torch._foreach_copy_(t[1:], [p.detach() for p in ps[1:]])
    dec = L.SdfDecoderC(t[1].data_ptr(), t[2].data_ptr(), t[3].data_ptr(), t[4].data_ptr(), d[0].out_features, float(d[0].activation.beta))
    r3 = s.radius3d_original
    fk = (r3.data_ptr(), r3._version, float(s.sdf_scale))
    if getattr(model, "_fac_cache", (None,))[0] != fk:
        model._fac_cache = (fk, (s.sdf_scale / r3).float().tolist())
    net = L.ColorNetC(*[x.data_ptr() for x in t[1:]], d[0].out_features, b[0].out_features, b[0].in_features, b[0].in_features - 54,
                      float(d[0].activation.beta), (ctypes.c_float * 3)(*model._fac_cache[1]))
    return t, dec, net, ps


def static_supported(model, cfg):
    qp = dict(model.ray_query_cfg.get("query_param", {}) or {})
    occ = getattr(getattr(model, "accel", None), "occ", None)
    return (getattr(model, "_color_fusable", lambda: False)() and model.use_view_dirs and occ is not None and occ.occ_grid.dim() == 3
            and occ.occ_grid.numel() * 4 // 32 <= 96 * 1024 and qp.get("num_coarse", 0) > 0 and len(qp.get("upsample_inv_s_factors", (1, 4, 16))) <= 4
            and qp.get("coarse_step_cfg", {}).get("step_mode", "linear") == "linear" and (cfg.get("with_rgb", True) or cfg.get("with_normal", True)))


def render_static(model, rays_o, rays_d, rays_h_appear=None, *, near=None, far=None, march_cap, kept_cap, coherent=False, with_rgb=True, with_normal=True,
                  perturb=False, training=None, depth_use_normalized_vw=True, cnt=None):
    P, lib = L.ptr, L.lib()
    if perturb:
        raise RuntimeError("render_static: perturb=True is not built (random streams of capacity-sized draws differ from the reference's); "
                           "use the host-sized path (SingleVolumeRenderer.render)")
    training = model.training if training is None else training
    R, dev = rays_o.shape[0], rays_o.device
    qp = dict(model.ray_query_cfg.get("query_param", {}) or {})
    nc1 = int(qp["num_coarse"]) + 1
    factors = list(qp.get("upsample_inv_s_factors", (1, 4, 16)))
    n_stage = len(factors)
    num_fine = qp.get("num_fine", 8)
    num_fine = [num_fine] * n_stage if isinstance(num_fine, int) else list(num_fine)
    num_fine = [n // 2 * 2 + 1 for n in num_fine]
    nf_tot = int(sum(num_fine))
    upsample_inv_s = qp.get("upsample_inv_s", 64.) / model.upsample_s_divisor
    use_est = bool(qp.get("upsample_use_estimate_alpha", False))
    nablas_has_grad = bool(qp.get("nablas_has_grad", False))
    mc = dict(qp.get("march_cfg", {}))
    fac = mc.pop("step_size_factor", 1.0)
    step_size, dt_gamma = mc.get("step_size", 1e-3) * fac, mc.get("dt_gamma", 0.0) * fac
    max_steps, max_step_size = int(mc.get("max_steps", 512)), mc.get("max_step_size", 1e10)
    march_cap, kept_cap = int(march_cap), int(kept_cap)
    S_cap = R * (nc1 + nf_tot)
    if cnt is None:
        cnt = torch.zeros(32, dtype=torch.int64, device=dev)
    else:
        cnt.zero_()
    st = _State()
    st.cnt = cnt
    wsb = (NF._scan_ws_bytes() + 255) // 256 * 256
    st.ws = torch.zeros(4, wsb, dtype=torch.uint8, device=dev)
    with torch.no_grad():
        t16, st.dec, st.net, masters = _fp16_images(model)
        st.held, st.grid16 = t16, t16[0]
        st.meta = model.implicit_surface.encoding.meta
        st.ml = model.implicit_surface._ml(model.max_level)
        st.collect = model.accel.occ.collect_struct() if training else None
        sp = model.space
        if getattr(sp, "_host_cr", None) is None or sp._host_cr[0] != (sp.aabb.data_ptr(), sp.aabb._version):
            c, r = sp.center.tolist(), sp.radius3d.tolist()
            sp._host_cr = ((sp.aabb.data_ptr(), sp.aabb._version), (ctypes.c_float * 3)(*c), (ctypes.c_float * 3)(*r))
        o_n, d_n = torch.empty(R, 3, device=dev), torch.empty(R, 3, device=dev)
        nr, fr = torch.empty(R, device=dev), torch.empty(R, device=dev)
        flag = torch.empty(R, dtype=torch.int32, device=dev)
        L.check(lib.nsb_ray_test_aabb(P(rays_o.contiguous(), "f32"), P(rays_d.contiguous(), "f32"), L.c_i64(R), sp._host_cr[1], sp._host_cr[2],
                                      ctypes.c_int(0 if near is None else 1), L.c_f32(0. if near is None else near),
                                      ctypes.c_int(0 if far is None else 1), L.c_f32(0. if far is None else far), P(o_n), P(d_n), P(nr), P(fr), P(flag),
                                      _slot(cnt, CNT_SLOTS["pairs"]), _slot(cnt, CNT_SLOTS["row_len"]), L.stream_ptr()), "ray_test_aabb")
        rays_inds = torch.empty(R, dtype=torch.int64, device=dev)
        _scan(flag, cnt, CNT_SLOTS["n_rays"], index=rays_inds, ws=st.ws[0])
        order_b = _block_order(rays_inds, None, R, cnt, CNT_SLOTS["n_rays"]) if coherent else None
        ha = rays_h_appear.detach().contiguous().float() if (rays_h_appear is not None and model.use_h_appear) else None
        if ha is None and model.use_h_appear:
            ha = torch.zeros(R, model.radiance_net.blocks.layers[0].in_features - 54, device=dev)
        n_ha = ha.shape[1] if ha is not None else 0
        rbuf = torch.zeros(R * (8 + n_ha), device=dev)
        o_c, d_c = rbuf[:3 * R].view(R, 3), rbuf[3 * R:6 * R].view(R, 3)
        n_c, f_c = rbuf[6 * R:7 * R], rbuf[7 * R:8 * R]
        ha_c = rbuf[8 * R:].view(R, n_ha) if ha is not None else None
        _call(lib.nsb_gather_rays, "gather_rays", cnt, CNT_SLOTS["n_rays"], None, P(rays_inds, "i64"), L.c_i64(R), P(o_n), P(d_n), P(nr), P(fr), P(o_c), P(d_c),
              P(n_c), P(f_c), P(ha, allow_none=True), P(ha_c, allow_none=True), L.c_i32(0 if ha is None else ha.shape[1]), L.stream_ptr())
        st.rays_o, st.rays_d = o_c, d_c
        view_dirs = (d_c / d_c.norm(dim=-1).clamp_min(1.0e-10).unsqueeze(-1)).contiguous()
        coarse = batch_sample_step_linear(n_c, f_c, nc1, prefix_shape=[R], perturb=perturb).contiguous()
        occ_grid = model.accel.occ.occ_grid
        res = occ_grid.shape[-3:]
        g8 = occ_grid.contiguous().view(torch.uint8)
        bits = torch.empty((occ_grid.numel() + 31) // 32, dtype=torch.int32, device=dev)
        L.check(lib.nsb_pack_occ_bits(P(g8, "u8"), L.c_i64(occ_grid.numel()), P(bits), L.stream_ptr()), "pack_occ_bits")
        roi = torch.tensor([-1, -1, -1, 1, 1, 1], dtype=torch.float32, device=dev) if getattr(model, "_static_roi", None) is None else model._static_roi
        model._static_roi = roi
        margs = (L.c_i64(R), P(o_c, "f32"), P(d_c, "f32"), P(n_c, "f32"), P(f_c, "f32"), P(roi, "f32"), None, L.c_i32(res[0]), L.c_i32(res[1]), L.c_i32(res[2]),
                 P(g8, "u8"), L.c_f32(step_size), L.c_f32(max_step_size), L.c_f32(dt_gamma), ctypes.c_uint32(max_steps))
        num_steps = torch.empty(R, dtype=torch.int32, device=dev)
        rec_t = torch.empty(R * max_steps, dtype=torch.float32, device=dev) if march_onepass(R, max_steps) else None
        with L.KERNEL_TIMER.time("march", R):
            if rec_t is not None:
                _call(lib.nsb_ray_marching_record, "ray_marching_record", cnt, CNT_SLOTS["n_rays"], None, L.c_i64(R), P(o_c, "f32"), P(d_c, "f32"), P(n_c, "f32"),
                      P(f_c, "f32"), P(roi, "f32"), L.c_i32(res[0]), L.c_i32(res[1]), L.c_i32(res[2]), P(g8, "u8"), L.c_f32(step_size), L.c_f32(max_step_size),
                      L.c_f32(dt_gamma), ctypes.c_uint32(max_steps), P(num_steps), P(rec_t), P(bits), L.stream_ptr())
            else:
                _call(lib.nsb_ray_marching_listed, "ray_marching", cnt, CNT_SLOTS["n_rays"], None, *margs, None, P(num_steps), None, None, None, None, None, None,
                      L.c_i64(0), P(bits), L.stream_ptr())
        info2 = torch.empty(R, 2, dtype=torch.int32, device=dev)
        ridx_hit = torch.empty(R, dtype=torch.int64, device=dev)
        pack_infos = torch.empty(R, 2, dtype=torch.int64, device=dev)
        _scan(num_steps, cnt, CNT_SLOTS["marched_raw"], info2=info2, index=ridx_hit, pack=pack_infos, ws=st.ws[1])
        _query_counts(cnt, 0, nc1, num_fine, march_cap, kept_cap)
        depth = torch.empty(march_cap, dtype=torch.float32, device=dev)
        ridx32 = torch.empty(march_cap, dtype=torch.int32, device=dev)
        with L.KERNEL_TIMER.time("march", R):
            if rec_t is not None:
                _call(lib.nsb_march_compact, "march_compact", cnt, CNT_SLOTS["hit"], None, P(rec_t, "f32"), ctypes.c_uint32(max_steps), P(info2, "i32"),
                      P(ridx_hit, "i64"), L.c_i64(R), P(depth), P(ridx32), L.stream_ptr())
            else:
                _call(lib.nsb_ray_marching_listed, "ray_marching", cnt, CNT_SLOTS["hit"], None, *margs, P(info2), None, P(depth), None, P(ridx32), None, None,
                      P(ridx_hit, "i64"), L.c_i64(R), P(bits), L.stream_ptr())
        ridx = ridx32.long()
        from . import neus as GN
        fine_stages = None
        if GN.use_persistent_upsample(R):
            fine_all, _ovf = NF.upsample_rays(st.meta, st.grid16, st.dec, ridx_hit, pack_infos, depth, o_c, d_c, [upsample_inv_s * f for f in factors], num_fine,
                                              max_level=st.ml, max_steps=max_steps, use_estimate_alpha=use_est, collect=st.collect, count=(cnt, CNT_SLOTS["hit"]))
            factors_loop = []
        else:
            factors_loop = factors
        sdf = torch.empty(march_cap if factors_loop else 1, dtype=torch.float32, device=dev)
        if factors_loop:
            fine_stages = []
            order_f = _block_order(rays_inds, ridx_hit, R, cnt, CNT_SLOTS["hit"]) if coherent and n_stage > 1 else None
            _sdf_launch(st.meta, st.grid16, st.dec, o_c, d_c, depth, sdf, ridx=ridx, ml=st.ml, collect=st.collect, cnt=cnt, slot=CNT_SLOTS["marched"])
        for i, factor in enumerate(factors_loop):
            cdf = torch.empty(march_cap, dtype=torch.float32, device=dev)
            _call(lib.nsb_neus_upsample_cdf, "neus_upsample_cdf", cnt, CNT_SLOTS["hit"], None, P(sdf, "f32"), P(depth, "f32"), P(pack_infos, "i64"), L.c_i64(R),
                  L.c_f32(upsample_inv_s * factor), ctypes.c_int(1 if use_est else 0), L.c_f32(1e-4), L.c_f32(0.0), P(cdf), L.stream_ptr())
            nf = num_fine[i]
            fine = torch.empty(R, nf, dtype=torch.float32, device=dev)
            u = NF._U_CACHE.get((nf, dev))
            if u is None:
                u = NF._U_CACHE[(nf, dev)] = torch.linspace(0., 1., nf + 2, device=dev, dtype=torch.float32)[1:-1].contiguous()
            _call(lib.nsb_packed_invert_cdf_shared_u, "packed_invert_cdf_shared_u", cnt, CNT_SLOTS["hit"], None, P(depth, "f32"), P(cdf, "f32"), P(u, "f32"),
                  P(pack_infos, "i64"), L.c_i64(R), L.c_i32(nf), P(fine), L.stream_ptr())
            fine_stages.append(fine)
            if i < n_stage - 1:
                sdf_fine = torch.empty(R * nf, dtype=torch.float32, device=dev)
                if coherent:
                    _sdf_launch(st.meta, st.grid16, st.dec, o_c, d_c, fine.view(-1), sdf_fine, packs=(get_pack_infos_from_batch(R, nf, device=dev), ridx_hit, order_f),
                                ml=st.ml, collect=st.collect, cnt=cnt, slot=CNT_SLOTS["hit"])
                else:
                    _sdf_launch(st.meta, st.grid16, st.dec, o_c, d_c, fine.view(-1), sdf_fine, ridx=ridx_hit.unsqueeze(-1).expand(R, nf).reshape(-1).contiguous(),
                                ml=st.ml, collect=st.collect, cnt=cnt, slot=CNT_SLOTS["fine0"] + i)
                dep_m = torch.empty(march_cap, dtype=torch.float32, device=dev)
                sdf_m = torch.empty(march_cap, dtype=torch.float32, device=dev)
                pim = torch.empty_like(pack_infos)
                _call(lib.nsb_merge_sorted_vals, "merge_sorted_vals", cnt, CNT_SLOTS["hit"], None, P(depth, "f32"), P(sdf, "f32"), P(pack_infos, "i64"),
                      P(fine, "f32"), P(sdf_fine, "f32"), L.c_i64(R), L.c_i32(nf), P(dep_m), P(sdf_m), P(pim), L.stream_ptr())
                depth, sdf, pack_infos = dep_m, sdf_m, pim
        if fine_stages is not None:
            fine_all = (torch.cat(fine_stages, dim=-1) if n_stage > 1 else fine_stages[0]).contiguous()
        d1 = torch.empty(S_cap, dtype=torch.float32, device=dev)
        mid = torch.empty(S_cap, dtype=torch.float32, device=dev)
        ridx_all = torch.empty(S_cap, dtype=torch.int64, device=dev)
        pinfo = torch.empty(R, 2, dtype=torch.int64, device=dev)
        rl = (ctypes.c_int32 * n_stage)(*num_fine)
        _call(lib.nsb_assemble_boundary, "assemble_boundary", cnt, CNT_SLOTS["n_rays"], CNT_SLOTS["hit"], P(coarse, "f32"), L.c_i64(R), L.c_i32(nc1),
              P(ridx_hit, "i64"), L.c_i64(R), P(fine_all, "f32"), L.c_i32(nf_tot), rl, L.c_i32(n_stage), P(d1), P(mid), P(ridx_all), P(pinfo), L.stream_ptr())
    s, b = model.implicit_surface, model.radiance_net.blocks.layers
    dl = s.decoder.layers
    sdf_b = _StaticSDF.apply(st, ridx_all, d1, (pinfo, None, order_b) if coherent else None, CNT_SLOTS["n_rays"] if coherent else CNT_SLOTS["boundary"],
                             s.encoding.flattened_params, dl[0].weight, dl[0].bias, dl[1].weight, dl[1].bias)
    inv_s = model.forward_inv_s()
    if not isinstance(inv_s, torch.Tensor):
        inv_s = torch.tensor(float(inv_s), device=dev)
    alpha, sel, steps = _StaticAlpha.apply(sdf_b, inv_s, pinfo, cnt, 1e-4, 0.0)
    with torch.no_grad():
        first = torch.empty(R, dtype=torch.int32, device=dev)
        nidx = torch.empty(R, dtype=torch.int64, device=dev)
        pinfo_kept = torch.empty(R, 2, dtype=torch.int64, device=dev)
        rays_inds_hit = torch.empty(R, dtype=torch.int64, device=dev)
        _scan(steps, cnt, CNT_SLOTS["kept_raw"], first=first, index=nidx, pack=pinfo_kept, src=rays_inds, nz_src=rays_inds_hit, ws=st.ws[2])
        _query_counts(cnt, 1, nc1, num_fine, march_cap, kept_cap)
        pidx, ridx_k = torch.empty(kept_cap, dtype=torch.int64, device=dev), torch.empty(kept_cap, dtype=torch.int64, device=dev)
        t_k, alpha_c = torch.empty(kept_cap, dtype=torch.float32, device=dev), torch.empty(kept_cap, dtype=torch.float32, device=dev)
        _call(lib.nsb_compact_samples, "compact_samples", cnt, CNT_SLOTS["rays_if_kept_fits"], None, P(sel.view(torch.uint8), "u8"), P(pinfo, "i64"), P(first, "i32"),
              P(steps, "i32"), L.c_i64(R), P(ridx_all, "i64"), P(mid, "f32"), P(alpha.detach(), "f32"), P(pidx), P(ridx_k), P(t_k), P(alpha_c), L.stream_ptr())
    alpha_k = _StaticGather.apply(alpha, pidx, alpha_c, cnt) if alpha.requires_grad else alpha_c
    params = (s.encoding.flattened_params, dl[0].weight, dl[0].bias, dl[1].weight, dl[1].bias, b[0].weight, b[0].bias, b[1].weight, b[1].bias,
              b[2].weight, b[2].bias)
    keep_acts = torch.is_grad_enabled() and any(p.requires_grad for p in params)
    _sdf_k, nab, rgb, x = _StaticColor.apply(st, ridx_k, t_k, view_dirs, ha_c, keep_acts, *params)
    if not nablas_has_grad:
        nab = nab.detach()
    nab_i = nab if with_normal else None
    if nab_i is not None and not training:
        nab_i = F.normalize(nab_i.clamp(-1, 1), dim=-1)
    vw, m, d, c, nn_ = _StaticComposite.apply(alpha_k, t_k, rgb if with_rgb else None, nab_i, pinfo_kept, rays_inds_hit, R, cnt,
                                              bool(depth_use_normalized_vw), 1e-4, 0.0)
    rendered = dict(mask_volume=m, depth_volume=d)
    if with_rgb:
        rendered["rgb_volume"] = c
    if with_normal:
        rendered["normals_volume"] = nn_
    buffers = dict(opacity_alpha=alpha_k, t=t_k, rgb=rgb, nablas=nab, net_x=x, vw=vw, pack_infos_hit=pinfo_kept, rays_inds_hit=rays_inds_hit, ridx=ridx_k,
                   pack_infos_boundary=pinfo, march_pack_infos=pack_infos)
    return rendered, cnt, buffers


def sliced_volume_buffer(buffers, cnt):
    c = cnt.tolist()
    K, Pu = c[CNT_SLOTS["kept"]], c[CNT_SLOTS["kept_rays"]]
    if c[CNT_SLOTS["overflow"]]:
        raise RuntimeError(f"static step: arena overflow (flags {c[CNT_SLOTS['overflow']]}: 1 = marched samples, 2 = kept samples)")
    if K == 0:
        return dict(type="empty", rays_inds_hit=[])
    vb = dict(type="packed", rays_inds_hit=buffers["rays_inds_hit"][:Pu], pack_infos_hit=buffers["pack_infos_hit"][:Pu])
    for k in ("opacity_alpha", "t", "rgb", "nablas", "net_x", "vw"):
        vb[k] = buffers[k][:K]
    return vb


class StaticFrame:

    def __init__(self, model, n_rays, loss_fn=None, *, near=None, far=None, with_rgb=True, with_normal=True, slack=1.5, march_cap=None, kept_cap=None,
                 coherent=None, use_graph=True, zero_grads=False, h_appear_dim=None, pre_hook=None):
        self.model, self.n_rays, self.loss_fn = model, int(n_rays), loss_fn
        self.near, self.far, self.with_rgb, self.with_normal, self.slack = near, far, with_rgb, with_normal, float(slack)
        self.march_cap, self.kept_cap, self.coherent = march_cap, kept_cap, coherent
        self.use_graph, self.zero_grads, self.pre_hook = use_graph, zero_grads, pre_hook
        dev = model.device
        self.device = dev
        self.rays_o = torch.zeros(self.n_rays, 3, device=dev)
        self.rays_d = torch.zeros(self.n_rays, 3, device=dev)
        na = h_appear_dim if h_appear_dim is not None else (model.radiance_net.blocks.layers[0].in_features - 54 if model.use_h_appear else 0)
        self.h_appear = torch.zeros(self.n_rays, na, device=dev) if na > 0 else None
        self.cnt = torch.zeros(32, dtype=torch.int64, device=dev)
        self.graph, self.loss, self.rendered, self.buffers, self._occ_captured = None, None, None, None, None
        self.captures = 0

    @torch.no_grad()
    def _probe(self):
        from ..renderer import SingleVolumeRenderer
        r = SingleVolumeRenderer(dict(near=self.near, far=self.far, with_rgb=self.with_rgb, with_normal=self.with_normal))
        r.train(self.model.training)
        out = r.ray_query(self.model, self.rays_o, self.rays_d, self.h_appear, return_buffer=True, return_details=True)
        det, vb = out.get("details", {}), out["volume_buffer"]
        qp = dict(self.model.ray_query_cfg.get("query_param", {}) or {})
        nf = qp.get("num_fine", 8)
        nf = [nf] * len(qp.get("upsample_inv_s_factors", (1, 4, 16))) if isinstance(nf, int) else list(nf)
        nf = [n // 2 * 2 + 1 for n in nf]
        M = int(det["march.num_per_ray"].sum()) if "march.num_per_ray" in det else 0
        n_hit = int(det["march.num_per_ray"].shape[0]) if "march.num_per_ray" in det else 0
        K = int(vb["t"].shape[0]) if vb.get("type") == "packed" else 0
        return M + n_hit * sum(nf[:-1]), K, bool(out["ray_tested"].get("rays_coherent", False))

    def _size(self, grow=1.0):
        need_m, need_k, coh = self._probe()
        if self.coherent is None:
            self.coherent = coh
        floor = 4096 + 8 * min(self.n_rays, 65536)
        m = int(max(need_m * self.slack, floor) * grow)
        k = int(max(need_k * self.slack, floor) * grow)
        self.march_cap = max(self.march_cap or 0, m)
        self.kept_cap = max(self.kept_cap or 0, k)

    def _run(self):
        if self.pre_hook is not None:
            self.pre_hook()
        if self.zero_grads:
            for p in self.model.parameters():
                if p.grad is not None:
                    p.grad.zero_()
        cv = getattr(self.model, "ctrl_var", None)
        if cv is not None and hasattr(cv, "mix_weight"):
            if getattr(cv, "_w_dev", None) is None:
                cv._w_dev = torch.zeros((), device=self.device)
            cv._use_w_dev = True
        try:
            rendered, _, buffers = render_static(self.model, self.rays_o, self.rays_d, self.h_appear, near=self.near, far=self.far, march_cap=self.march_cap,
                                                 kept_cap=self.kept_cap, coherent=bool(self.coherent), with_rgb=self.with_rgb, with_normal=self.with_normal, cnt=self.cnt)
        finally:
            if cv is not None:
                cv._use_w_dev = False
        loss = None
        if self.loss_fn is not None:
            loss = self.loss_fn(rendered)
            if loss.requires_grad:
                loss.backward()
            loss = loss.detach()
        return rendered, buffers, loss

    def capture(self):
        if self.march_cap is None or self.kept_cap is None or self.coherent is None:
            self._size()
        if not self.use_graph:
            self.graph = None
            return self
        if not bool(self.rays_d.any()):
            raise RuntimeError("StaticFrame.capture: the input buffers hold no rays yet; call step(rays_o, rays_d, ...) or fill frame.rays_o / frame.rays_d first")
        was = L.KERNEL_TIMER.enabled
        L.KERNEL_TIMER.enabled = False
        import gc
        gc.collect()
        try:
            side = torch.cuda.Stream(device=self.device)
            side.wait_stream(torch.cuda.current_stream())
            with torch.cuda.stream(side):
                for _ in range(2):
                    self._run()
            torch.cuda.current_stream().wait_stream(side)
            torch.cuda.synchronize()
            g = torch.cuda.CUDAGraph()
            self._occ_captured = self.model.accel.occ.occ_grid
            with torch.cuda.graph(g, stream=side):
                self.rendered, self.buffers, self.loss = self._run()
            self.graph = g
            self.captures += 1
        finally:
            L.KERNEL_TIMER.enabled = was
        return self

    def step(self, rays_o, rays_d, rays_h_appear=None):
        self.rays_o.copy_(rays_o, non_blocking=True)
        self.rays_d.copy_(rays_d, non_blocking=True)
        if self.h_appear is not None and rays_h_appear is not None:
            self.h_appear.copy_(rays_h_appear, non_blocking=True)
        cv = getattr(self.model, "ctrl_var", None)
        if cv is not None and hasattr(cv, "mix_weight"):
            if getattr(cv, "_w_dev", None) is None:
                cv._w_dev = torch.zeros((), device=self.device)
            cv._w_dev.fill_(cv.mix_weight())
        if self.graph is None and (self.use_graph or self.march_cap is None):
            self.capture()
        if self.graph is not None:
            occ = self.model.accel.occ.occ_grid
            if self._occ_captured is not None and occ.data_ptr() != self._occ_captured.data_ptr():
                self._occ_captured.copy_(occ)
            self.graph.replay()
        else:
            self.rendered, self.buffers, self.loss = self._run()
        return self.loss

    def counts(self):
        c = self.cnt.tolist()
        return {k: c[v] for k, v in CNT_SLOTS.items()}

    def check(self, retry=True):
        if int(self.cnt[CNT_SLOTS["overflow"]]) == 0:
            return True
        self.march_cap = self.kept_cap = None
        self._size(grow=1.25)
        self.graph = None
        if self.use_graph:
            self.capture()
        if retry:
            if self.graph is not None:
                self.graph.replay()
            else:
                self.rendered, self.buffers, self.loss = self._run()
        return False

    def volume_buffer(self):
        return sliced_volume_buffer(self.buffers, self.cnt)
```

Baseline: 27.77.

## Recompute color MLP activations in backward instead of storing Z, Y1, Y2 tiles

```diff
diff --git a/neuralsim_b200/csrc/color_tc.cu b/neuralsim_b200/csrc/color_tc.cu
--- a/neuralsim_b200/csrc/color_tc.cu
+++ b/neuralsim_b200/csrc/color_tc.cu
@@ -24,18 +24,11 @@
 }
 
 
-__device__ __forceinline__ void level_jacobian(const PLMeta &m, uint32_t p, const float (&xs)[3], const __half *__restrict__ grid,
-                                               float (&J0)[3], float (&J1)[3]) {
-    uint32_t cell[8];
-    float w[8], fr[3], scale[3];
-    level_cells3(m, p, xs, cell, w, fr, scale);
-    const uint32_t *lp = level_cells_ptr(m, p, grid);
+__device__ __forceinline__ void level_jacobian_cells(const uint32_t (&raw)[8], const float (&fr)[3], const float (&scale)[3], float (&J0)[3],
+                                                     float (&J1)[3]) {
     float2 v[8];
 #pragma unroll
-    for (int c = 0; c < 8; ++c) {
-        const uint32_t raw = ld_nc_u32(lp + cell[c]);
-        v[c] = __half22float2(*reinterpret_cast<const __half2 *>(&raw));
-    }
+    for (int c = 0; c < 8; ++c) v[c] = __half22float2(*reinterpret_cast<const __half2 *>(&raw[c]));
 #pragma unroll
     for (int gd = 0; gd < 3; ++gd) {
         float a0 = 0.f, a1 = 0.f;
@@ -57,6 +50,14 @@
         J1[gd] = a1;
     }
 }
+__device__ __forceinline__ void level_jacobian(const PLMeta &m, uint32_t p, const float (&xs)[3], const __half *__restrict__ grid,
+                                               float (&J0)[3], float (&J1)[3]) {
+    uint32_t cell[8], raw[8];
+    float w[8], fr[3], scale[3];
+    level_cells3(m, p, xs, cell, w, fr, scale);
+    level_load_cells(level_cells_ptr(m, p, grid), cell, raw);
+    level_jacobian_cells(raw, fr, scale, J0, J1);
+}
 
 __device__ __forceinline__ void unpack8(const uint4 &q, float (&v)[8]) {
     const __half2 *h = reinterpret_cast<const __half2 *>(&q);
@@ -66,30 +67,11 @@
 
 constexpr int kColorGatherU = 4;
 
+constexpr int kColorFwdCtasPerSM = 3;
 constexpr int kColorBwdCtasPerSM = 2;
 
-__global__ void __launch_bounds__(kTile)
-k_color_fwd(const PLMeta m, const __half *__restrict__ grid, const ColorNetDev net, const PointSrc ps, const float *__restrict__ view_dirs,
-            const float *__restrict__ h_appear, int64_t n, int max_level, float *__restrict__ sdf_out, float *__restrict__ nab_out,
-            float *__restrict__ rgb_out, float *__restrict__ x_out, uint8_t *__restrict__ Zt, uint8_t *__restrict__ Xt,
-            uint8_t *__restrict__ Y1t, uint8_t *__restrict__ Y2t, const OccCollect oc, const int64_t *__restrict__ n_dev) {
-    n = eff_n(n, n_dev);
-    extern __shared__ uint8_t dyn_smem[];
-    uint8_t *tiles = reinterpret_cast<uint8_t *>((reinterpret_cast<uintptr_t>(dyn_smem) + 1023) & ~uintptr_t(1023));
-    uint8_t *sX = tiles;
-    uint8_t *sU = sX + kTileBytes;
-    uint8_t *sW1 = sU + kTileBytes;
-    uint8_t *sW1T = sW1 + HW * NF * 2;
-    uint8_t *sR1 = sW1T + HW * NF * 2;
-    uint8_t *sR2 = sR1 + XW * XW * 2;
-    constexpr int kS = tc::acc_stride(64);
-    float *acc = reinterpret_cast<float *>(sR2 + XW * XW * 2);
-    __shared__ float sb1[HW], sW2[HW], srb1[XW], srb2[XW], sR3[3][XW];
-    __shared__ float sb2, srb3[3];
-
-    const int tid = threadIdx.x;
-    stage_W1(net.dec, sW1, tid);
-    stage_W1T(net.dec, sW1T, tid);
+__device__ __forceinline__ void stage_radiance(const ColorNetDev &net, uint8_t *sR1, uint8_t *sR2, float *srb1, float *srb2, float (*sR3)[XW],
+                                               int tid) {
     for (int e = tid; e < XW * XW; e += kTile) {
         const int j = e % XW, k = e / XW;
         const int rc = ref_col(k, net.n_appear);
@@ -98,13 +80,55 @@
         *reinterpret_cast<__half *>(sR1 + (k / 8) * (XW * 16) + j * 16 + (k % 8) * 2) = v1;
         *reinterpret_cast<__half *>(sR2 + (k / 8) * (XW * 16) + j * 16 + (k % 8) * 2) = v2;
     }
-    stage_decoder_vectors(net.dec, sb1, sW2, &sb2, tid);
     if (tid < XW) {
         srb1[tid] = tid < net.rw ? __half2float(net.rb1[tid]) : 0.f;
         srb2[tid] = tid < net.rw ? __half2float(net.rb2[tid]) : 0.f;
 #pragma unroll
         for (int k = 0; k < 3; ++k) sR3[k][tid] = tid < net.rw ? __half2float(net.R3[k * net.rw + tid]) : 0.f;
     }
+}
+
+template <int N>
+__device__ __forceinline__ void bias_round_to_tile(const float (&d)[2][N / 2], const float *bias, bool relu, uint8_t *tile) {
+#pragma unroll
+    for (int h = 0; h < 2; ++h)
+#pragma unroll
+        for (int c = 0; c < N / 8; ++c)
+#pragma unroll
+            for (int r = 0; r < 2; ++r) {
+                const int col = tc::frag_col(c);
+                float v[2];
+#pragma unroll
+                for (int j = 0; j < 2; ++j) {
+                    v[j] = r16(bias ? d[h][4 * c + 2 * r + j] + bias[col + j] : d[h][4 * c + 2 * r + j]);
+                    if (relu) v[j] = fmaxf(v[j], 0.f);
+                }
+                tc::st_pair_f16(tile, tc::pair_off<kTile>(h * 64 + tc::frag_row(r), col), v[0], v[1]);
+            }
+}
+
+__global__ void __launch_bounds__(kTile, kColorFwdCtasPerSM)
+k_color_fwd(const PLMeta m, const __half *__restrict__ grid, const ColorNetDev net, const PointSrc ps, const float *__restrict__ view_dirs,
+            const float *__restrict__ h_appear, int64_t n, int max_level, float *__restrict__ sdf_out, float *__restrict__ nab_out,
+            float *__restrict__ rgb_out, float *__restrict__ x_out, uint8_t *__restrict__ Xt, const OccCollect oc, const int64_t *__restrict__ n_dev) {
+    n = eff_n(n, n_dev);
+    extern __shared__ uint8_t dyn_smem[];
+    uint8_t *tiles = reinterpret_cast<uint8_t *>((reinterpret_cast<uintptr_t>(dyn_smem) + 1023) & ~uintptr_t(1023));
+    uint8_t *sX = tiles;
+    uint8_t *sU = sX + kTileBytes;
+    uint8_t *sS = sU + kTileBytes;
+    uint8_t *sW1 = sS + kTileBytes;
+    uint8_t *sW1T = sW1 + HW * NF * 2;
+    uint8_t *sR1 = sW1T + HW * NF * 2;
+    uint8_t *sR2 = sR1 + XW * XW * 2;
+    __shared__ float sb1[HW], sW2[HW], srb1[XW], srb2[XW], sR3[3][XW];
+    __shared__ float sb2, srb3[3];
+
+    const int tid = threadIdx.x;
+    stage_W1(net.dec, sW1, tid);
+    stage_W1T(net.dec, sW1T, tid);
+    stage_radiance(net, sR1, sR2, srb1, srb2, sR3, tid);
+    stage_decoder_vectors(net.dec, sb1, sW2, &sb2, tid);
     if (tid == 0) {
         for (int k = 0; k < 3; ++k) srb3[k] = __half2float(net.rb3[k]);
     }
@@ -124,42 +148,47 @@
         gather_row_to_tile<kTile, kColorGatherU>(m, grid, xs, max_level, sX, tid);
         tc::fence_async_smem();
         __syncthreads();
-        tc::mma_to_rows<64, 0, 0, NF / 16>(acc, kS, 0, tc::kmajor(x_addr, kTile), tc::kmajor(w1_addr, HW), false);
+        {
+            float z[2][HW / 2];
+            tc::mma_m128<HW, 0, 0, NF / 16>(z, tc::kmajor(x_addr, kTile), tc::kmajor(w1_addr, HW), false);
+            bias_round_to_tile<HW>(z, sb1, false, sS);
+        }
         __syncthreads();
         float out = 0.f;
-        uint8_t *zt = Zt ? Zt + tile * kTileBytes : nullptr;
 #pragma unroll 1
         for (int c = 0; c < HW / 8; ++c) {
             float z[8], uu[8];
-            tc::acc_ld8(acc, kS, tid, c * 8, z);
+            unpack8(*reinterpret_cast<const uint4 *>(sS + c * kChunk + tid * 16), z);
 #pragma unroll
             for (int j = 0; j < 8; ++j) {
-                z[j] = r16(z[j] + sb1[c * 8 + j]);
                 float a, s;
                 softplus_as(z[j], spk, a, s);
                 out = fmaf(r16(a), sW2[c * 8 + j], out);
                 uu[j] = sW2[c * 8 + j] * s;
             }
             *reinterpret_cast<uint4 *>(sU + c * kChunk + tid * 16) = tc::pack8_f16(uu);
-            if (zt) *reinterpret_cast<uint4 *>(zt + c * kChunk + tid * 16) = tc::pack8_f16(z);
         }
         const float sdf = r16(out + sb2);
         tc::fence_async_smem();
         __syncthreads();
-        tc::mma_to_rows<32, 0, 0, HW / 16>(acc, kS, 0, tc::kmajor(u_addr, kTile), tc::kmajor(w1t_addr, NF), false);
+        {
+            float g[2][NF / 2];
+            tc::mma_m128<NF, 0, 0, HW / 16>(g, tc::kmajor(u_addr, kTile), tc::kmajor(w1t_addr, NF), false);
+            bias_round_to_tile<NF>(g, nullptr, false, sS);
+        }
         __syncthreads();
         float nacc[3] = {0.f, 0.f, 0.f};
 #pragma unroll 1
         for (uint32_t g4 = 0; g4 < 4; ++g4) {
             float gg[8];
-            tc::acc_ld8(acc, kS, tid, g4 * 8, gg);
+            unpack8(*reinterpret_cast<const uint4 *>(sS + g4 * kChunk + tid * 16), gg);
 #pragma unroll
             for (uint32_t q = 0; q < 4; ++q) {
                 const uint32_t p = g4 * 4 + q;
                 if ((int)m.level[p] <= max_level) {
                     float J0[3], J1[3];
                     level_jacobian(m, p, xs, grid, J0, J1);
-                    const float g0 = r16(gg[2 * q]), g1 = r16(gg[2 * q + 1]);
+                    const float g0 = gg[2 * q], g1 = gg[2 * q + 1];
 #pragma unroll
                     for (int d = 0; d < 3; ++d) nacc[d] = __fmaf_rn(g0, J0[d], nacc[d]);
 #pragma unroll
@@ -201,36 +230,25 @@
         }
         tc::fence_async_smem();
         __syncthreads();
-        tc::mma_to_rows<64, 0, 0, XW / 16>(acc, kS, 0, tc::kmajor(x_addr, kTile), tc::kmajor(r1_addr, XW), false);
-        __syncthreads();
-        uint8_t *y1t = Y1t ? Y1t + tile * kTileBytes : nullptr;
+        {
+            float y[2][XW / 2];
+            tc::mma_m128<XW, 0, 0, XW / 16>(y, tc::kmajor(x_addr, kTile), tc::kmajor(r1_addr, XW), false);
+            bias_round_to_tile<XW>(y, srb1, true, sU);
+            tc::fence_async_smem();
+            __syncthreads();
+            tc::mma_m128<XW, 0, 0, XW / 16>(y, tc::kmajor(u_addr, kTile), tc::kmajor(r2_addr, XW), false);
+            bias_round_to_tile<XW>(y, srb2, true, sS);
+        }
+        __syncthreads();
+        float o3[3] = {0.f, 0.f, 0.f};
 #pragma unroll 1
         for (int c = 0; c < XW / 8; ++c) {
             float y[8];
-            tc::acc_ld8(acc, kS, tid, c * 8, y);
-#pragma unroll
-            for (int j = 0; j < 8; ++j) y[j] = fmaxf(r16(y[j] + srb1[c * 8 + j]), 0.f);
-            const uint4 q = tc::pack8_f16(y);
-            *reinterpret_cast<uint4 *>(sU + c * kChunk + tid * 16) = q;
-            if (y1t) *reinterpret_cast<uint4 *>(y1t + c * kChunk + tid * 16) = q;
-        }
-        tc::fence_async_smem();
-        __syncthreads();
-        tc::mma_to_rows<64, 0, 0, XW / 16>(acc, kS, 0, tc::kmajor(u_addr, kTile), tc::kmajor(r2_addr, XW), false);
-        __syncthreads();
-        float o3[3] = {0.f, 0.f, 0.f};
-        uint8_t *y2t = Y2t ? Y2t + tile * kTileBytes : nullptr;
-#pragma unroll 1
-        for (int c = 0; c < XW / 8; ++c) {
-            float y[8];
-            tc::acc_ld8(acc, kS, tid, c * 8, y);
-#pragma unroll
-            for (int j = 0; j < 8; ++j) {
-                y[j] = fmaxf(r16(y[j] + srb2[c * 8 + j]), 0.f);
+            unpack8(*reinterpret_cast<const uint4 *>(sS + c * kChunk + tid * 16), y);
+#pragma unroll
+            for (int j = 0; j < 8; ++j)
 #pragma unroll
                 for (int k = 0; k < 3; ++k) o3[k] = fmaf(y[j], sR3[k][c * 8 + j], o3[k]);
-            }
-            if (y2t) *reinterpret_cast<uint4 *>(y2t + c * kChunk + tid * 16) = tc::pack8_f16(y);
         }
         if (valid) {
             sdf_out[i] = sdf;
@@ -248,9 +266,8 @@
 }
 
 __global__ void __launch_bounds__(kTile, kColorBwdCtasPerSM)
-k_color_rad_bwd(const ColorNetDev net, const uint8_t *__restrict__ Xt, const uint8_t *__restrict__ Y1t, const uint8_t *__restrict__ Y2t,
-                const float *__restrict__ rgb, const float *__restrict__ g_rgb, int64_t n, float *__restrict__ dh_out,
-                float *__restrict__ dR1, float *__restrict__ drb1, float *__restrict__ dR2, float *__restrict__ drb2,
+k_color_rad_bwd(const ColorNetDev net, const uint8_t *__restrict__ Xt, const float *__restrict__ rgb, const float *__restrict__ g_rgb, int64_t n,
+                float *__restrict__ dh_out, float *__restrict__ dR1, float *__restrict__ drb1, float *__restrict__ dR2, float *__restrict__ drb2,
                 float *__restrict__ dR3, float *__restrict__ drb3, const int64_t *__restrict__ n_dev) {
     n = eff_n(n, n_dev);
     constexpr int NE = 80;
@@ -259,27 +276,14 @@
     uint8_t *sT = tiles;
     uint8_t *sY1 = sT + 3 * kTileBytes;
     uint8_t *sXe = sY1 + kTile * NE * 2;
-    uint8_t *sR2T = sXe + kTile * NE * 2;
-    uint8_t *sR1h = sR2T + XW * XW * 2;
-    __shared__ float sR3[3][XW];
+    uint8_t *sR1 = sXe + kTile * NE * 2;
+    uint8_t *sR2 = sR1 + XW * XW * 2;
+    __shared__ float srb1[XW], srb2[XW], sR3[3][XW];
     __shared__ float sdb3[3];
     __shared__ __align__(8) uint64_t mbar_ld;
 
     const int tid = threadIdx.x, lane = tid & 31;
-    for (int e = tid; e < XW * XW; e += kTile) {
-        const int i = e % XW, j = e / XW;
-        const __half v = (j < net.rw && i < net.rw) ? net.R2[j * net.rw + i] : __float2half_rn(0.f);
-        *reinterpret_cast<__half *>(sR2T + (j / 8) * (XW * 16) + i * 16 + (j % 8) * 2) = v;
-    }
-    for (int e = tid; e < NF * XW; e += kTile) {
-        const int k = e % NF, j = e / NF;
-        const __half v = j < net.rw ? net.R1[j * net.rin + 22 + k] : __float2half_rn(0.f);
-        *reinterpret_cast<__half *>(sR1h + (j / 8) * (NF * 16) + k * 16 + (j % 8) * 2) = v;
-    }
-    if (tid < XW) {
-#pragma unroll
-        for (int k = 0; k < 3; ++k) sR3[k][tid] = tid < net.rw ? __half2float(net.R3[k * net.rw + tid]) : 0.f;
-    }
+    stage_radiance(net, sR1, sR2, srb1, srb2, sR3, tid);
     *reinterpret_cast<uint4 *>(sY1 + 8 * kChunk + tid * 16) = make_uint4(0x00003C00u, 0, 0, 0);
     *reinterpret_cast<uint4 *>(sY1 + 9 * kChunk + tid * 16) = make_uint4(0, 0, 0, 0);
     *reinterpret_cast<uint4 *>(sXe + 9 * kChunk + tid * 16) = make_uint4(0, 0, 0, 0);
@@ -296,23 +300,19 @@
     tc::fence_async_smem();
     __syncthreads();
     const uint32_t t_addr = tc::smem_u32(sT), y1_addr = tc::smem_u32(sY1), xe_addr = tc::smem_u32(sXe);
-    const uint32_t r2t_addr = tc::smem_u32(sR2T), r1h_addr = tc::smem_u32(sR1h);
+    const uint32_t r1_addr = tc::smem_u32(sR1), r2_addr = tc::smem_u32(sR2);
     uint32_t ld_phase = 0;
     bool first_tile = true;
 
     const int64_t n_tiles = (n + kTile - 1) / kTile;
     auto fetch = [&](int64_t tile) {
-        tc::mbar_arrive_expect_tx(&mbar_ld, 3 * kTileBytes);
-        tc::tma_load_bulk(sT + 2 * kTileBytes, Y2t + tile * kTileBytes, kTileBytes, &mbar_ld);
-        tc::tma_load_bulk(sY1, Y1t + tile * kTileBytes, kTileBytes, &mbar_ld);
+        tc::mbar_arrive_expect_tx(&mbar_ld, kTileBytes);
         tc::tma_load_bulk(sXe, Xt + tile * kTileBytes, kTileBytes, &mbar_ld);
     };
     if (tid == 0 && (int64_t)blockIdx.x < n_tiles) fetch(blockIdx.x);
     for (int64_t tile = blockIdx.x; tile < n_tiles; tile += gridDim.x) {
         const int64_t i = tile * kTile + tid;
         const bool valid = i < n;
-        tc::mbar_wait(&mbar_ld, ld_phase);
-        ld_phase ^= 1;
         float gy[3] = {0.f, 0.f, 0.f};
         if (valid && g_rgb) {
 #pragma unroll
@@ -330,6 +330,20 @@
             const float sgy = warp_sum(gy[k]);
             if (lane == 0 && sgy != 0.f) atomicAdd(&sdb3[k], sgy);
         }
+        tc::mbar_wait(&mbar_ld, ld_phase);
+        ld_phase ^= 1;
+        tc::fence_async_smem();
+        __syncthreads();
+        {
+            float y[2][XW / 2];
+            tc::mma_m128<XW, 0, 0, XW / 16>(y, tc::kmajor(xe_addr, kTile), tc::kmajor(r1_addr, XW), false);
+            bias_round_to_tile<XW>(y, srb1, true, sY1);
+            tc::fence_async_smem();
+            __syncthreads();
+            tc::mma_m128<XW, 0, 0, XW / 16>(y, tc::kmajor(y1_addr, kTile), tc::kmajor(r2_addr, XW), false);
+            bias_round_to_tile<XW>(y, srb2, true, sT + 2 * kTileBytes);
+        }
+        __syncthreads();
 #pragma unroll 1
         for (int c = 0; c < 8; ++c) {
             float y2[8], d[8];
@@ -345,7 +359,7 @@
         __syncthreads();
         {
             float dy[2][XW / 2];
-            tc::mma_m128<64, 0, 0, XW / 16>(dy, tc::kmajor(t_addr, kTile), tc::kmajor(r2t_addr, XW), false);
+            tc::mma_m128<64, 0, 1, XW / 16>(dy, tc::kmajor(t_addr, kTile), tc::mnmajor(r2_addr, XW), false);
 #pragma unroll
             for (int h = 0; h < 2; ++h)
 #pragma unroll
@@ -360,7 +374,7 @@
         tc::fence_async_smem();
         __syncthreads();
         float dh[2][NF / 2];
-        tc::mma_m128<32, 0, 0, XW / 16>(dh, tc::kmajor(t_addr + kTileBytes, kTile), tc::kmajor(r1h_addr, NF), false);
+        tc::mma_m128<32, 0, 1, XW / 16>(dh, tc::kmajor(t_addr + kTileBytes, kTile), tc::mnmajor(r1_addr, XW), false);
         tc::mma_m64<NE, 1, 1, kTile / 16>(xa, tc::mnmajor(t_addr, kTile), tc::mnmajor(y1_addr, kTile), true);
         tc::mma_m64<NE, 1, 1, kTile / 16>(xb, tc::mnmajor(t_addr + kTileBytes, kTile), tc::mnmajor(xe_addr, kTile), true);
         tc::mma_m64<8, 1, 1, kTile / 16>(x3, tc::mnmajor(t_addr + 2 * kTileBytes, kTile), tc::mnmajor(xe_addr + 8 * kChunk, kTile), true);
@@ -413,10 +427,9 @@
 }
 
 __global__ void __launch_bounds__(kTile, kColorBwdCtasPerSM)
-k_color_sdf_bwd(const PLMeta m, const __half *__restrict__ grid, const ColorNetDev net, const PointSrc ps, const uint8_t *__restrict__ Zt,
-                const uint8_t *__restrict__ Xt, const float *__restrict__ g_nab, const float *__restrict__ g_sdf, const float *__restrict__ dh_r,
-                int64_t n, int max_level, float *__restrict__ d_grid, float *__restrict__ d_W1, float *__restrict__ d_b1, float *__restrict__ d_W2,
-                float *__restrict__ d_b2, const int64_t *__restrict__ n_dev) {
+k_color_sdf_bwd(const PLMeta m, const __half *__restrict__ grid, const ColorNetDev net, const PointSrc ps, const float *__restrict__ g_nab,
+                const float *__restrict__ g_sdf, const float *__restrict__ dh_r, int64_t n, int max_level, float *__restrict__ d_grid,
+                float *__restrict__ d_W1, float *__restrict__ d_b1, float *__restrict__ d_W2, float *__restrict__ d_b2, const int64_t *__restrict__ n_dev) {
     n = eff_n(n, n_dev);
     constexpr int NX = 48;
     extern __shared__ uint8_t dyn_smem[];
@@ -426,18 +439,16 @@
     uint8_t *sGe = sHe + kTile * NX * 2;
     uint8_t *sW1 = sGe + kTile * NX * 2;
     uint8_t *sW1T = sW1 + HW * NF * 2;
-    uint8_t *sZ = sW1T + NF * HW * 2;
     constexpr int kS = tc::acc_stride(2 * NF);
     float *stage = reinterpret_cast<float *>(sT);
     static_assert(kTile * kS * 4 <= 3 * kTileBytes, "the staged rows must fit in T");
-    __shared__ float sW2[HW], sdsdf[kTile];
+    __shared__ float sb1[HW], sW2[HW], sdsdf[kTile];
     __shared__ float sdb2;
-    __shared__ __align__(8) uint64_t mbar_ld;
 
     const int tid = threadIdx.x, lane = tid & 31;
     stage_W1(net.dec, sW1, tid);
     stage_W1T(net.dec, sW1T, tid);
-    stage_decoder_vectors(net.dec, nullptr, sW2, nullptr, tid);
+    stage_decoder_vectors(net.dec, sb1, sW2, nullptr, tid);
     *reinterpret_cast<uint4 *>(sHe + 4 * kChunk + tid * 16) = make_uint4(0x00003C00u, 0, 0, 0);
     *reinterpret_cast<uint4 *>(sGe + 4 * kChunk + tid * 16) = make_uint4(0x00003C00u, 0, 0, 0);
     *reinterpret_cast<uint4 *>(sHe + 5 * kChunk + tid * 16) = make_uint4(0, 0, 0, 0);
@@ -447,26 +458,15 @@
     for (int k = 0; k < NX / 2; ++k) wacc[k] = 0.f;
 #pragma unroll
     for (int k = 0; k < 4; ++k) vacc[k] = 0.f;
-    if (tid == 0) {
-        sdb2 = 0.f;
-        tc::mbar_init(&mbar_ld, 1);
-        tc::fence_mbar_init();
-    }
+    if (tid == 0) sdb2 = 0.f;
     tc::fence_async_smem();
     __syncthreads();
     const uint32_t t_addr = tc::smem_u32(sT), he_addr = tc::smem_u32(sHe), ge_addr = tc::smem_u32(sGe), w1_addr = tc::smem_u32(sW1),
                    w1t_addr = tc::smem_u32(sW1T);
     const SoftplusK spk(net.dec.beta);
-    uint32_t ld_phase = 0;
     bool first_tile = true;
 
     const int64_t n_tiles = (n + kTile - 1) / kTile;
-    auto fetch = [&](int64_t tile) {
-        tc::mbar_arrive_expect_tx(&mbar_ld, kTileBytes + 4 * kChunk);
-        tc::tma_load_bulk(sZ, Zt + tile * kTileBytes, kTileBytes, &mbar_ld);
-        tc::tma_load_bulk(sHe, Xt + tile * kTileBytes, 4 * kChunk, &mbar_ld);
-    };
-    if (tid == 0 && (int64_t)blockIdx.x < n_tiles) fetch(blockIdx.x);
     for (int64_t tile = blockIdx.x; tile < n_tiles; tile += gridDim.x) {
         const int64_t i = tile * kTile + tid;
         const bool valid = i < n;
@@ -480,41 +480,31 @@
         }
         const float dsdf = (valid && g_sdf) ? g_sdf[i] : 0.f;
         sdsdf[tid] = dsdf;
-        tc::mbar_wait(&mbar_ld, ld_phase);
-        ld_phase ^= 1;
-#pragma unroll 1
-        for (int c = 0; c < 8; ++c) {
-            float z[8], uu[8];
-            unpack8(*reinterpret_cast<const uint4 *>(sZ + c * kChunk + tid * 16), z);
-#pragma unroll
-            for (int j = 0; j < 8; ++j) {
-                float a, s;
-                softplus_as(z[j], spk, a, s);
-                uu[j] = sW2[c * 8 + j] * s;
-            }
-            *reinterpret_cast<uint4 *>(sT + kTileBytes + c * kChunk + tid * 16) = tc::pack8_f16(uu);
-        }
 #pragma unroll 4
         for (uint32_t p = 0; p < 16; ++p) {
-            uint32_t packed = 0;
+            uint32_t hp = 0, packed = 0;
             if ((int)m.level[p] <= max_level) {
-                float J0[3], J1[3];
-                level_jacobian(m, p, xs, grid, J0, J1);
+                uint32_t cell[8], raw[8];
+                float w[8], fr[3], sc[3], J0[3], J1[3];
+                level_cells3(m, p, xs, cell, w, fr, sc);
+                level_load_cells(level_cells_ptr(m, p, grid), cell, raw);
+                hp = level_interp2(raw, w);
+                level_jacobian_cells(raw, fr, sc, J0, J1);
                 float a0 = 0.f, a1 = 0.f;
 #pragma unroll
                 for (int d = 0; d < 3; ++d) { a0 = __fmaf_rn(gin[d], J0[d], a0); a1 = __fmaf_rn(gin[d], J1[d], a1); }
                 const __half2 h = __floats2half2_rn(a0, a1);
                 packed = *reinterpret_cast<const uint32_t *>(&h);
             }
+            *reinterpret_cast<uint32_t *>(sHe + (p >> 2) * kChunk + tid * 16 + (p & 3) * 4) = hp;
             *reinterpret_cast<uint32_t *>(sGe + (p >> 2) * kChunk + tid * 16 + (p & 3) * 4) = packed;
         }
         tc::fence_async_smem();
         __syncthreads();
-        float gfr[2][NF / 2];
-        {
-            float du[2][HW / 2];
-            tc::mma_m128<64, 0, 0, NF / 16>(du, tc::kmajor(ge_addr, kTile), tc::kmajor(w1_addr, HW), false);
-            tc::mma_m128<32, 0, 0, HW / 16>(gfr, tc::kmajor(t_addr + kTileBytes, kTile), tc::kmajor(w1t_addr, NF), false);
+        {
+            float zf[2][HW / 2], du[2][HW / 2];
+            tc::mma_m128<HW, 0, 0, NF / 16>(zf, tc::kmajor(he_addr, kTile), tc::kmajor(w1_addr, HW), false);
+            tc::mma_m128<HW, 0, 0, NF / 16>(du, tc::kmajor(ge_addr, kTile), tc::kmajor(w1_addr, HW), false);
 #pragma unroll
             for (int h = 0; h < 2; ++h)
 #pragma unroll
@@ -525,26 +515,28 @@
                     for (int c = 0; c < HW / 8; ++c) {
                         const int col = tc::frag_col(c);
                         const uint32_t off = tc::pair_off<kTile>(row, col);
-                        const float2 z2 = tc::ld_pair_f16(sZ, off);
-                        float dz[2], vv[2];
+                        float uu[2], dz[2], vv[2];
 #pragma unroll
                         for (int j = 0; j < 2; ++j) {
-                            const float z = j ? z2.y : z2.x;
+                            const float z = r16(zf[h][4 * c + 2 * r + j] + sb1[col + j]);
                             float a, s;
                             softplus_as(z, spk, a, s);
                             const float w2 = sW2[col + j], d = r16(du[h][4 * c + 2 * r + j]);
                             const float curv = (z * spk.k > spk.thr) ? 0.f : spk.beta * s * (1.f - s);
+                            uu[j] = w2 * s;
                             dz[j] = d * w2 * curv + ds * w2 * s;
                             vv[j] = d * s + ds * r16(a);
                         }
                         tc::st_pair_f16(sT, off, dz[0], dz[1]);
+                        tc::st_pair_f16(sT + kTileBytes, off, uu[0], uu[1]);
                         tc::st_pair_f16(sT + 2 * kTileBytes, off, vv[0], vv[1]);
                     }
                 }
         }
         tc::fence_async_smem();
         __syncthreads();
-        float dhz[2][NF / 2];
+        float gfr[2][NF / 2], dhz[2][NF / 2];
+        tc::mma_m128<32, 0, 0, HW / 16>(gfr, tc::kmajor(t_addr + kTileBytes, kTile), tc::kmajor(w1t_addr, NF), false);
         tc::mma_m128<32, 0, 0, HW / 16>(dhz, tc::kmajor(t_addr, kTile), tc::kmajor(w1t_addr, NF), false);
         tc::mma_m64<NX, 1, 1, kTile / 16>(wacc, tc::mnmajor(t_addr, kTile), tc::mnmajor(he_addr, kTile), true);
         tc::mma_m64<NF, 1, 1, kTile / 16>(*reinterpret_cast<float(*)[NF / 2]>(wacc), tc::mnmajor(t_addr + kTileBytes, kTile), tc::mnmajor(ge_addr, kTile), true);
@@ -553,10 +545,6 @@
         const float dsum = warp_sum(dsdf);
         if (lane == 0 && dsum != 0.f) atomicAdd(&sdb2, dsum);
         __syncthreads();
-        if (tid == 0 && tile + gridDim.x < n_tiles) {
-            tc::fence_async_smem();
-            fetch(tile + gridDim.x);
-        }
         tc::frag_store<NF>(gfr, stage, kS, 0);
         tc::frag_store<NF>(dhz, stage, kS, NF);
         __syncthreads();
@@ -651,22 +639,22 @@
                                    const float *rays_d, const int64_t *ridx, const float *t, const float *view_dirs, const float *h_appear,
                                    int64_t n, int32_t max_level, float *sdf, float *nablas, float *rgb, float *x_out, void *act_z, void *act_x,
                                    void *act_y1, void *act_y2, const nsb_occ_collect *collect, void *stream) {
+    (void)act_z; (void)act_y1; (void)act_y2;
     const DevCounts dn = take_counts();
     if (n == 0) return 0;
     NSB_REQUIRE(meta && params_half && net && sdf && nablas && rgb && view_dirs, "nsb_fused_color_fwd: NULL argument");
     NSB_REQUIRE(x || (rays_o && rays_d && t), "nsb_fused_color_fwd: need x or (rays_o, rays_d, t)");
-    NSB_REQUIRE((act_z && act_x && act_y1 && act_y2) || (!act_z && !act_x && !act_y1 && !act_y2), "nsb_fused_color_fwd: pass all four activation buffers or none");
     PLMeta m;
     ColorNetDev d;
     if (int rc = make_net(net, meta, &m, &d, "nsb_fused_color_fwd")) return rc;
     NSB_REQUIRE(d.n_appear == 0 || h_appear, "nsb_fused_color_fwd: h_appear is NULL but the net has %d appearance channels", d.n_appear);
-    constexpr int kSmem = 2 * kTileBytes + 2 * HW * NF * 2 + 2 * XW * XW * 2 + kTile * tc::acc_stride(64) * 4 + 1024;
+    constexpr int kSmem = 3 * kTileBytes + 2 * HW * NF * 2 + 2 * XW * XW * 2 + 1024;
     opt_in_smem(k_color_fwd, kSmem);
+    if (int rc = require_ctas_per_sm(k_color_fwd, kTile, kSmem, kColorFwdCtasPerSM, "nsb_fused_color_fwd")) return rc;
     const PointSrc ps{x, rays_o, rays_d, t, ridx};
-    k_color_fwd<<<persistent_grid(n_tiles(n), 2), kTile, kSmem, (cudaStream_t)stream>>>(m, (const __half *)params_half, d, ps, view_dirs, h_appear, n,
-                                                                                        max_level < 0 ? -1 : max_level, sdf, nablas, rgb, x_out, (uint8_t *)act_z,
-                                                                                        (uint8_t *)act_x, (uint8_t *)act_y1, (uint8_t *)act_y2,
-                                                                                        occ_collect_of(collect), dn.a);
+    k_color_fwd<<<persistent_grid(n_tiles(n), kColorFwdCtasPerSM), kTile, kSmem, (cudaStream_t)stream>>>(
+        m, (const __half *)params_half, d, ps, view_dirs, h_appear, n, max_level < 0 ? -1 : max_level, sdf, nablas, rgb, x_out, (uint8_t *)act_x,
+        occ_collect_of(collect), dn.a);
     return check_launch("nsb_fused_color_fwd");
 }
 
@@ -678,7 +666,8 @@
                                    void *stream) {
     const DevCounts dn = take_counts();
     if (n == 0) return 0;
-    NSB_REQUIRE(meta && params_half && net && act_z && act_x && act_y1 && act_y2 && rgb && dh_scratch, "nsb_fused_color_bwd: NULL argument");
+    (void)act_z; (void)act_y1; (void)act_y2;
+    NSB_REQUIRE(meta && params_half && net && act_x && rgb && dh_scratch, "nsb_fused_color_bwd: NULL argument");
     NSB_REQUIRE(d_grid && d_W1 && d_b1 && d_W2 && d_b2 && d_R1 && d_rb1 && d_R2 && d_rb2 && d_R3 && d_rb3, "nsb_fused_color_bwd: NULL gradient buffer");
     NSB_REQUIRE(x || (rays_o && rays_d && t), "nsb_fused_color_bwd: need x or (rays_o, rays_d, t)");
     PLMeta m;
@@ -687,20 +676,19 @@
     cudaStream_t s = (cudaStream_t)stream;
     const float *dh = nullptr;
     if (g_rgb) {
-        constexpr int kSmemR = 3 * kTileBytes + 2 * kTile * 80 * 2 + XW * XW * 2 + NF * XW * 2 + 1024;
+        constexpr int kSmemR = 3 * kTileBytes + 2 * kTile * 80 * 2 + 2 * XW * XW * 2 + 1024;
         opt_in_smem(k_color_rad_bwd, kSmemR);
         if (int rc = require_ctas_per_sm(k_color_rad_bwd, kTile, kSmemR, kColorBwdCtasPerSM, "nsb_fused_color_bwd(radiance)")) return rc;
-        k_color_rad_bwd<<<persistent_grid(n_tiles(n), kColorBwdCtasPerSM), kTile, kSmemR, s>>>(d, (const uint8_t *)act_x, (const uint8_t *)act_y1,
-                                                                                               (const uint8_t *)act_y2, rgb, g_rgb, n, dh_scratch, d_R1,
+        k_color_rad_bwd<<<persistent_grid(n_tiles(n), kColorBwdCtasPerSM), kTile, kSmemR, s>>>(d, (const uint8_t *)act_x, rgb, g_rgb, n, dh_scratch, d_R1,
                                                                                                d_rb1, d_R2, d_rb2, d_R3, d_rb3, dn.a);
         if (int rc = check_launch("nsb_fused_color_bwd(radiance)")) return rc;
         dh = dh_scratch;
     }
-    constexpr int kSmemS = 3 * kTileBytes + 2 * kTile * 48 * 2 + 2 * HW * NF * 2 + kTileBytes + 1024;
+    constexpr int kSmemS = 3 * kTileBytes + 2 * kTile * 48 * 2 + 2 * HW * NF * 2 + 1024;
     opt_in_smem(k_color_sdf_bwd, kSmemS);
     if (int rc = require_ctas_per_sm(k_color_sdf_bwd, kTile, kSmemS, kColorBwdCtasPerSM, "nsb_fused_color_bwd(sdf)")) return rc;
     const PointSrc ps{x, rays_o, rays_d, t, ridx};
-    k_color_sdf_bwd<<<persistent_grid(n_tiles(n), kColorBwdCtasPerSM), kTile, kSmemS, s>>>(m, (const __half *)params_half, d, ps, (const uint8_t *)act_z, (const uint8_t *)act_x,
-                                                                          g_nablas, g_sdf, dh, n, max_level < 0 ? -1 : max_level, d_grid, d_W1, d_b1, d_W2, d_b2, dn.a);
+    k_color_sdf_bwd<<<persistent_grid(n_tiles(n), kColorBwdCtasPerSM), kTile, kSmemS, s>>>(m, (const __half *)params_half, d, ps, g_nablas, g_sdf, dh, n,
+                                                                                           max_level < 0 ? -1 : max_level, d_grid, d_W1, d_b1, d_W2, d_b2, dn.a);
     return check_launch("nsb_fused_color_bwd(sdf)");
 }
diff --git a/neuralsim_b200/csrc/fused_tc_common.cuh b/neuralsim_b200/csrc/fused_tc_common.cuh
--- a/neuralsim_b200/csrc/fused_tc_common.cuh
+++ b/neuralsim_b200/csrc/fused_tc_common.cuh
@@ -44,7 +44,11 @@
 #pragma unroll
         for (int u = 0; u < U; ++u) level_cells3(m, p0 + u, xs, cell[u], w[u]);
 #pragma unroll
-        for (int u = 0; u < U; ++u) packed[u] = level_feat2_cells(level_cells_ptr(m, p0 + u, grid), cell[u], w[u]);
+        for (int u = 0; u < U; ++u) {
+            uint32_t raw[8];
+            level_load_cells(level_cells_ptr(m, p0 + u, grid), cell[u], raw);
+            packed[u] = level_interp2(raw, w[u]);
+        }
 #pragma unroll
         for (int u = 0; u < U; ++u) {
             const uint32_t p = p0 + u;
diff --git a/neuralsim_b200/csrc/lotd_device.cuh b/neuralsim_b200/csrc/lotd_device.cuh
--- a/neuralsim_b200/csrc/lotd_device.cuh
+++ b/neuralsim_b200/csrc/lotd_device.cuh
@@ -201,10 +201,11 @@
     return q;
 }
 
-__device__ __forceinline__ uint32_t level_feat2_cells(const uint32_t *__restrict__ lp, const uint32_t (&cell)[8], const float (&w)[8]) {
-    uint32_t raw[8];
+__device__ __forceinline__ void level_load_cells(const uint32_t *__restrict__ lp, const uint32_t (&cell)[8], uint32_t (&raw)[8]) {
 #pragma unroll
     for (int c = 0; c < 8; ++c) raw[c] = ld_nc_u32(lp + cell[c]);
+}
+__device__ __forceinline__ uint32_t level_interp2(const uint32_t (&raw)[8], const float (&w)[8]) {
     __half2 acc = __floats2half2_rn(0.f, 0.f);
 #pragma unroll
     for (int c = 0; c < 8; ++c) {
diff --git a/neuralsim_b200/fields/fused_color.py b/neuralsim_b200/fields/fused_color.py
--- a/neuralsim_b200/fields/fused_color.py
+++ b/neuralsim_b200/fields/fused_color.py
@@ -19,14 +19,11 @@
         nab = torch.empty(n, 3, dtype=torch.float32, device=dev)
         rgb = torch.empty(n, 3, dtype=torch.float32, device=dev)
         x = torch.empty(n, 3, dtype=torch.float32, device=dev)
-        acts = None
-        if keep:
-            acts = torch.empty(4, int(L.lib().nsb_color_tile_bytes(L.c_i64(n))), dtype=torch.uint8, device=dev)
-        ap = [L.ptr(acts[k]) if keep else None for k in range(4)]
+        acts = torch.empty(int(L.lib().nsb_color_tile_bytes(L.c_i64(n))), dtype=torch.uint8, device=dev) if keep else None
         with L.KERNEL_TIMER.time("fused_color_fwd", n):
             L.check(L.lib().nsb_fused_color_fwd(meta.c_ref, L.ptr(grid16, "f16"), ctypes.byref(net), None, L.ptr(rays_o, "f32"), L.ptr(rays_d, "f32"),
                                                 L.ptr(ridx, "i64"), L.ptr(t, "f32"), L.ptr(view_dirs, "f32"), L.ptr(h_appear, "f32", allow_none=True),
-                                                L.c_i64(n), L.c_i32(max_level), L.ptr(sdf), L.ptr(nab), L.ptr(rgb), L.ptr(x), *ap,
+                                                L.c_i64(n), L.c_i32(max_level), L.ptr(sdf), L.ptr(nab), L.ptr(rgb), L.ptr(x), None, L.ptr(acts, allow_none=True), None, None,
                                                 ctypes.byref(collect) if collect is not None else None, L.stream_ptr()),
                     "fused_color_fwd")
         ctx.model, ctx.pts, ctx.max_level, ctx.n = model, pts, max_level, n
@@ -58,9 +55,8 @@
         dh = torch.empty(n, 32, dtype=torch.float32, device=dev)
         with L.KERNEL_TIMER.time("fused_color_bwd", n):
             L.check(L.lib().nsb_fused_color_bwd(meta.c_ref, L.ptr(grid16, "f16"), ctypes.byref(net), None, L.ptr(rays_o, "f32"), L.ptr(rays_d, "f32"),
-                                                L.ptr(ridx, "i64"), L.ptr(t, "f32"), L.c_i64(n), L.c_i32(ctx.max_level), L.ptr(acts[0]), L.ptr(acts[1]),
-                                                L.ptr(acts[2]), L.ptr(acts[3]), L.ptr(rgb), L.ptr(g_sdf, allow_none=True), L.ptr(g_nab, allow_none=True),
-                                                L.ptr(g_rgb, allow_none=True), L.ptr(dh), *[L.ptr(g) for g in grads], L.stream_ptr()),
+                                                L.ptr(ridx, "i64"), L.ptr(t, "f32"), L.c_i64(n), L.c_i32(ctx.max_level), None, L.ptr(acts), None, None, L.ptr(rgb),
+                                                L.ptr(g_sdf, allow_none=True), L.ptr(g_nab, allow_none=True), L.ptr(g_rgb, allow_none=True), L.ptr(dh), *[L.ptr(g) for g in grads], L.stream_ptr()),
                     "fused_color_bwd")
         return (None,) * 7 + tuple(grads)
 
diff --git a/neuralsim_b200/graphics/neus_static.py b/neuralsim_b200/graphics/neus_static.py
--- a/neuralsim_b200/graphics/neus_static.py
+++ b/neuralsim_b200/graphics/neus_static.py
@@ -168,13 +168,12 @@
         nab = torch.empty(n, 3, dtype=torch.float32, device=dev)
         rgb = torch.empty(n, 3, dtype=torch.float32, device=dev)
         x = torch.empty(n, 3, dtype=torch.float32, device=dev)
-        acts = torch.empty(4, int(L.lib().nsb_color_tile_bytes(L.c_i64(n))), dtype=torch.uint8, device=dev) if keep_acts else None
-        ap = [L.ptr(acts[k]) if keep_acts else None for k in range(4)]
+        acts = torch.empty(int(L.lib().nsb_color_tile_bytes(L.c_i64(n))), dtype=torch.uint8, device=dev) if keep_acts else None
         P = L.ptr
         with L.KERNEL_TIMER.time("fused_color_fwd", n):
             _call(L.lib().nsb_fused_color_fwd, "fused_color_fwd", st.cnt, CNT_SLOTS["kept"], None,
                   st.meta.c_ref, P(st.grid16, "f16"), ctypes.byref(st.net), None, P(st.rays_o, "f32"), P(st.rays_d, "f32"), P(ridx, "i64"), P(t, "f32"),
-                  P(view_dirs, "f32"), P(h_appear, "f32", allow_none=True), L.c_i64(n), L.c_i32(st.ml), P(sdf), P(nab), P(rgb), P(x), *ap,
+                  P(view_dirs, "f32"), P(h_appear, "f32", allow_none=True), L.c_i64(n), L.c_i32(st.ml), P(sdf), P(nab), P(rgb), P(x), None, P(acts, allow_none=True), None, None,
                   ctypes.byref(st.collect) if st.collect is not None else None, L.stream_ptr())
         ctx.st, ctx.ridx, ctx.t, ctx.n = st, ridx, t, n
         ctx.held = (acts, rgb)
@@ -205,7 +204,7 @@
         with L.KERNEL_TIMER.time("fused_color_bwd", n):
             _call(L.lib().nsb_fused_color_bwd, "fused_color_bwd", st.cnt, CNT_SLOTS["kept"], None,
                   st.meta.c_ref, P(st.grid16, "f16"), ctypes.byref(st.net), None, P(st.rays_o, "f32"), P(st.rays_d, "f32"), P(ctx.ridx, "i64"),
-                  P(ctx.t, "f32"), L.c_i64(n), L.c_i32(st.ml), P(acts[0]), P(acts[1]), P(acts[2]), P(acts[3]), P(rgb), P(g_sdf, allow_none=True),
+                  P(ctx.t, "f32"), L.c_i64(n), L.c_i32(st.ml), None, P(acts), None, None, P(rgb), P(g_sdf, allow_none=True),
                   P(g_nab, allow_none=True), P(g_rgb, allow_none=True), P(dh), *[P(g) for g in grads], L.stream_ptr())
         return (None,) * 6 + tuple(grads)
 
```

Measured after the change: 27.86, median of 6. About the same (+0.3%).
